# KohakuBlueleaf/UwUDiff

Measured on AMD Instinct MI355X. Metric: train images/sec (whole node), DiT-S/2 256^2 latent, higher is better.
Workload: dtype bf16; 1 GPU; DiT-S/2 (L12 D384 h6), 4x32x32 synthetic latents + pooled-text cond 1280, eps-MSE, AdamW lr1e-6 wd0.01 cosine; random-init weights; per_gpu_batch=768, global_batch=768, parallelism=dp1

## Files before the change

include/uwu_hip.h:

```cpp
#ifndef UWU_HIP_H
#define UWU_HIP_H

#include <stddef.h>
#include <stdint.h>

#ifdef __cplusplus
extern "C" {
#endif

#define UWU_F32 0
#define UWU_BF16 1

#define UWU_OK 0
#define UWU_EINVAL (-1)
#define UWU_ELAUNCH (-2)
#define UWU_ENOTIMPL (-3)

#define UWU_PT_EPSILON 0
#define UWU_PT_V 1
#define UWU_PT_SAMPLE 2
#define UWU_PT_RF 3

#define UWU_EPI_NONE 0
#define UWU_EPI_BIAS 1
#define UWU_EPI_BIAS_GELU 2
#define UWU_EPI_DGELU 3
#define UWU_EPI_BIAS_SILU 4
#define UWU_EPI_ACCUM 5

const char* uwu_last_error(void);
int uwu_version(void);
int uwu_env_refresh(void);
int uwu_memset_zero(void* p, uint64_t bytes, void* stream);


int uwu_schedule_gather(const int64_t* timesteps, const float* sigmas_desc, const float* all_snr,
                        const float* alphas_cumprod, int n_train, int B, int snr_mode, float gamma,
                        int debias, float* coef, void* stream);

int uwu_rf_time_to_sigma(const float* u01, float sigma_max, const float* log_sigmas_asc, int n_train,
                         int B, float* coef, float* timesteps, void* stream);

int uwu_qsample(const float* x, const float* noise, const float* coef, int B, int64_t n, float* noisy,
                void* noisy_bf16, void* stream);

int uwu_qsample_norm(const float* x, const float* noise, const float* coef, int B, int64_t n, float vae_mean,
                     float vae_std, float* x_norm, float* noisy, void* stream);

int uwu_philox_raw(uint32_t* out, int64_t n_counters, uint64_t seed, uint64_t offset, void* stream);
int uwu_philox_normal(float* out, int64_t n, uint64_t seed, uint64_t offset, void* stream);
int uwu_draw_timesteps(int64_t* timesteps, int n_train, int B, uint64_t seed, uint64_t offset, void* stream);
int uwu_draw_u01(float* u01, int B, uint64_t seed, uint64_t offset, void* stream);
int uwu_qsample_draw(const float* x, const float* coef, int B, int64_t n, int use_norm, float vae_mean, float vae_std,
                     float* x_norm, float* noise, float* noisy, uint64_t seed, uint64_t offset, void* stream);
int uwu_posterior_draw(const float* moments, int ldm, int B, int latent, int64_t HW, float* z, float* mean_out, float* logvar_out,
                       uint64_t seed, uint64_t offset, void* stream);

int uwu_ctx_place(const void* src, int dtype, const int64_t* mask, float* out, int B, int S, int F, int S_total,
                  int F_total, int s_off, int f_off, void* stream);

int uwu_loss_fwd_bwd(const float* x, const float* noise, const float* xt, const void* model_output,
                     int out_dtype, const float* coef, int pred_type, int target_type, int force_convert,
                     int B, int64_t n, float* losses, float* loss_mean, void* grad_out, float* pred,
                     float* target, void* stream);

int uwu_scale_inplace(void* y, int dtype, int64_t n, const float* scale, void* stream);
int uwu_scale_into(const void* x, void* y, int dtype, int64_t n, const float* scale, void* stream);
int uwu_cast_i64_to_f32(const int64_t* x, float* y, int64_t n, void* stream);

int uwu_aggregate_concat(const void* emb, const int* starts, void* out, int B, int max_n, int64_t unit_bytes,
                         int elem_size, uint64_t pad_bits, void* stream);
int uwu_aggregate_split(const void* cat, const int* starts, void* out, int B, int max_n, int64_t unit_bytes,
                        void* stream);
int uwu_aggregate_first(const void* emb, const int* starts, void* out, int B, int64_t unit_bytes, void* stream);

int uwu_sampler_step(const float* x, const float* eps_cond, const float* eps_uncond, const float* noise, float* out,
                     float* denoised, int64_t n, float cfg, float sigma, float sigma_down, float sigma_up,
                     float s_noise, void* stream);
int uwu_sampler_combine(const float* base, const float* eps_cond, const float* eps_uncond, const float* noise,
                        float* out, int64_t n, float cfg, float a, float b, float c, void* stream);
int uwu_scale_copy(const float* x, float* y, int64_t n, float scale, void* stream);

int uwu_cfg_input(const float* x, float* y, int B, int64_t n, float c_in, void* stream);
int uwu_sampler_combine_draw(const float* base, const float* eps_cond, const float* eps_uncond, float* out, int64_t n, float cfg,
                             float a, float b, float c, uint64_t seed, uint64_t offset, void* stream);
size_t uwu_latent_finish_ws_bytes(int B, int64_t n);
int uwu_latent_finish(const float* x, float* y, int B, int64_t n, int rescale, float vae_std, float vae_mean, void* ws,
                      size_t ws_bytes, void* stream);
int uwu_image_u8(const void* x, int dtype, void* y, int B, int H, int W, void* stream);


int uwu_grad_sqnorm_clip(const float* g, int64_t n, float pre_scale, float max_norm, float* partial,
                         float* out, void* stream);

int uwu_adamw_step(float* p, float* g, float* m, float* v, void* p_bf16, int64_t n, float lr,
                   float beta1, float beta2, float eps, float weight_decay, int step, float pre_scale,
                   const float* clip, int zero_grad, void* stream);

int uwu_cast_f32_to_bf16(const float* src, void* dst, int64_t n, void* stream);
int uwu_cast_bf16_to_f32(const void* src, float* dst, int64_t n, void* stream);

#define UWU_ADAPTER_NORM 0
#define UWU_ADAPTER_LORA 1
#define UWU_ADAPTER_LOKR 2
#define UWU_ADAPTER_LOKR_LOWRANK 3
int uwu_adapter_merge(const float* base, const float* p, const int64_t* table, const int64_t* blk_start, int nseg,
                      int64_t nblocks, float* eff, void* shadow, void* stream);
int uwu_adapter_grad(const float* dw, int64_t N, int64_t K, int kind, const float* p, float* g, int64_t pa, int64_t pb,
                     int64_t pc, int r, int out_k, int in_n, float scale, float* ws, int64_t ws_elems, void* stream);

int uwu_comm_unique_id(void* id128);
int uwu_comm_init(const void* id128, int rank, int world, void** comm);
int uwu_allreduce_flat(void* comm, float* buf, int64_t n, void* stream);
int uwu_comm_destroy(void* comm);


int uwu_gemm(const void* A, const void* B, void* C, void* C2, const float* bias, const void* aux,
             int M, int N, int K, int lda, int ldb, int ldc, int ldaux, int transA, int transB, int dtype,
             int c_dtype, int epilogue, int split_k, void* stream);

#define UWU_FP8_E4M3 0
#define UWU_FP8_E5M2 1
size_t uwu_gemm_fp8_scratch_bytes(int M, int N, int K);
int uwu_gemm_fp8(const void* A, const void* B, void* C, void* C2, const float* bias, const void* aux, int M, int N,
                 int K, int lda, int ldb, int ldc, int ldaux, int fmt_a, int epilogue, const float* scale_a,
                 const float* scale_b, void* scratch, size_t scratch_bytes, void* stream);

int uwu_gemm_fp8_emit(const void* A, const void* B, void* C, float* colsum, const float* bias, const void* aux, int M, int N,
                      int K, int lda, int ldb, int ldc, int ldaux, int fmt_a, int epilogue, const float* scale_a,
                      const float* scale_b, void* q8, int ldq, void* q8t, int ldqt, const float* q_scale, float* q_amax,
                      void* stream);

int uwu_conv3x3_implicit_ok(int B, int H, int W, int C, int Cout, int stride, int dtype);
int uwu_conv3x3_fwd(const void* x, const void* w, const float* bias, void* y, int B, int H, int W, int C, int Cout,
                    int stride, int dtype, void* stream);
size_t uwu_conv3x3_s2br_ws_bytes(int B, int H, int W, int C, int Cout, int dtype);
int uwu_conv3x3_s2br_fwd(const void* x, const void* w, const float* bias, void* y, int B, int H, int W, int C, int Cout, int dtype,
                         void* ws, size_t ws_bytes, void* stream);
int uwu_conv3x3_dgrad(const void* dy, const void* w, void* dx, int B, int H, int W, int C, int Cout, int stride, int dtype,
                      void* stream);
size_t uwu_conv3x3_wgrad_scratch_bytes(int C, int Cout, int64_t Mo);
int uwu_conv3x3_wgrad(const void* dy, const void* x, float* dw, float* db, int B, int H, int W, int C, int Cout, int stride,
                      int dtype, void* scratch, size_t scratch_bytes, void* stream);

int uwu_fp8_amax(const void* x, int dtype, int64_t n, float* amax, void* stream);
int uwu_fp8_update_scales(float* amax, float* scale, const int* fmt, int n, float margin, void* stream);
int uwu_fp8_quantize(const void* x, int dtype, int M, int K, int ldx, const float* scale, int fmt, void* out, int ldo,
                     void* out_t, int ldt, float* amax, float* colsum, void* stream);

size_t uwu_gemm_wgrad_scratch_bytes(int M, int N, int K);
int uwu_gemm_wgrad(const void* A, const void* B, float* C, float* bias_grad, int M, int N, int K, int lda, int ldb,
                   int ldc, int dtype, int blocks, void* scratch, size_t scratch_bytes, void* stream);

size_t uwu_gemm_wgrad_pair_scratch_bytes(int M_a, int N_a, int M_b, int N_b, int K);
int uwu_gemm_wgrad_pair(const void* A_a, const void* B_a, float* C_a, float* bias_grad_a, int M_a, int N_a, int lda_a,
                        int ldb_a, int ldc_a, const void* A_b, const void* B_b, float* C_b, float* bias_grad_b, int M_b,
                        int N_b, int lda_b, int ldb_b, int ldc_b, int K, int dtype, int blocks, void* scratch,
                        size_t scratch_bytes, void* stream);

int uwu_gemm_prof_enable(int on);
int uwu_gemm_prof_collect(int kind, double* ms, double* flops, int* launches);

enum {
  UWU_PROF_GEMM_FWD = 0, UWU_PROF_GEMM_DGRAD = 1, UWU_PROF_GEMM_WGRAD = 2, UWU_PROF_GEMM_FC1_GELU = 3,
  UWU_PROF_GEMM_FC2_DGELU = 4, UWU_PROF_ATTN_FWD = 5, UWU_PROF_ATTN_BWD = 6, UWU_PROF_LN_FWD = 7, UWU_PROF_LN_BWD = 8,
  UWU_PROF_CONV = 9, UWU_PROF_OTHER = 10
};
int uwu_prof_enable(int on);
int uwu_prof_collect(int tag, int kind, double* ms, double* flops, double* bytes, int* launches);

int uwu_colsum(const void* X, int dtype, int M, int N, int ldx, float* out, int accumulate, void* stream);

int uwu_skinny_linear_ok(int M, int N, int K);
int uwu_skinny_linear_fwd(const float* X, const float* W, const float* bias, float* Y, float* Y2, int M, int N, int K,
                          int epilogue, void* stream);
int uwu_skinny_linear_dgrad(const float* dY, const float* W, float* dX, int M, int N, int K, void* stream);
int uwu_skinny_linear_wgrad(const float* dY, const float* X, float* dW, float* db, int M, int N, int K, void* stream);
int uwu_colsum_batched(const void* X, int dtype, int batch, int M, int N, int ldx, float* out, int accumulate,
                       void* stream);


int uwu_add_ln_modulate_fwd(const void* x_in, const void* y, const float* gate, const float* shift,
                            const float* scale, int mod_ld, void* x_out, void* h, float* mean, float* rstd,
                            int B, int T, int D, float eps, int affine, int dtype, void* stream);
int uwu_add_ln_modulate_fwd_q8(const void* x_in, const void* y, const float* gate, const float* shift, const float* scale,
                               int mod_ld, void* x_out, void* q8, int ldq, void* q8t, int ldqt, const float* q_scale,
                               float* q_amax, float* mean, float* rstd, int B, int T, int D, float eps, void* stream);


int uwu_add_ln_modulate_bwd(const void* dh, const void* x, const float* mean, const float* rstd,
                            const float* scale, const void* dx_in, const void* y, const float* gate,
                            int mod_ld, void* dx_out, void* dy, float* dshift, float* dscale, float* dgate,
                            int B, int T, int D, int affine, int dtype, void* stream);


int uwu_attention_fwd(const void* q, const void* k, const void* v, void* o, float* lse, int B, int Tq, int Tk,
                      int H, int d, int ldq, int ldk, int ldv, int ldo, float scale, int dtype, void* stream);
int uwu_attention_d512_fwd(const void* q, const void* k, const void* v, void* o, int B, int T, int ldq, int ldk, int ldv, int ldo,
                           float scale, int dtype, void* stream);
int uwu_attention_causal_fwd(const void* q, const void* k, const void* v, const int64_t* key_mask, void* o, int B, int T, int H,
                             int d, int ldq, int ldk, int ldv, int ldo, float scale, int dtype, void* stream);
int uwu_text_embed(const int64_t* ids, const void* tok_table, const void* pos_table, void* out, int B, int T, int D, int vocab,
                   int dtype, void* stream);
#define UWU_ACT_QUICK_GELU 0
#define UWU_ACT_GELU_ERF 1
int uwu_bias_act_fwd(const void* x, const float* bias, void* y, int M, int N, int ld, int kind, int dtype, void* stream);
int uwu_text_pool(const int64_t* ids, const void* h, void* pooled, int B, int T, int D, int eos_id, int dtype, void* stream);
int uwu_attention_relbias_fwd(const void* q, const void* k, const void* v, const float* rel_bias, const int64_t* key_mask, void* o,
                              int B, int T, int H, int d, int ldq, int ldk, int ldv, int ldo, float scale, int dtype, void* stream);
int uwu_add_rmsnorm_fwd(const void* x_in, const void* y, const float* weight, void* x_out, void* n_out, int M, int D, float eps,
                        int dtype, void* stream);
#define UWU_GATE_GELU_TANH 0
int uwu_gated_act_fwd(const void* u, void* out, int M, int F, int ldu, int ldo, int kind, int dtype, void* stream);
int uwu_t5_rel_bias(const float* weight, const int32_t* bucket, float* out, int num_buckets, int H, int n, void* stream);
int uwu_token_embed(const int64_t* ids, const void* tok_table, void* out, int B, int T, int D, int vocab, int dtype, void* stream);
int uwu_attention_bwd(const void* q, const void* k, const void* v, const void* o, const void* dO,
                      const float* lse, float* delta, void* dq, void* dk, void* dv, int B, int Tq, int Tk, int H,
                      int d, int ldq, int ldk, int ldv, int ldo, float scale, int dtype, void* stream);
int uwu_attention_bias_fwd(const void* q, const void* k, const void* v, const float* key_bias, void* o, float* lse,
                           int B, int Tq, int Tk, int H, int d, int ldq, int ldk, int ldv, int ldo, float scale,
                           int dtype, void* stream);
int uwu_attention_bias_bwd(const void* q, const void* k, const void* v, const float* key_bias, const void* o,
                           const void* dO, const float* lse, float* delta, void* dq, void* dk, void* dv, int B,
                           int Tq, int Tk, int H, int d, int ldq, int ldk, int ldv, int ldo, float scale, int dtype,
                           void* stream);

int uwu_axial_rope_fwd(const void* x, const float* pos, const float* fh, const float* fw, void* y, int64_t rows,
                       int H, int d, int ldx, int dtype, void* stream);
int uwu_axial_rope_bwd(const void* x, const void* dy, const float* pos, const float* fh, const float* fw, void* dx,
                       float* dfh, float* dfw, int64_t rows, int H, int d, int ldx, int dtype, void* stream);

int uwu_axial_rope_bwd_shared(const void* x, const void* dy, const float* pos, int pos_rows, const float* fh, const float* fw,
                              void* dx, float* dfh, float* dfw, int64_t rows, int H, int d, int ldx, int dtype, void* stream);
int uwu_axial_rope_table(const float* pos, const float* fh, const float* fw, float* tab, int T, int H, int d, int ldt,
                         void* stream);
int uwu_attention_rope_fwd(const void* q, const void* k, const void* v, const float* rope_tab, void* o, float* lse, int B,
                           int T, int H, int d, int ldq, int ldk, int ldv, int ldo, int ldt, float scale, int dtype,
                           void* stream);
int uwu_attention_rope_bwd(const void* q, const void* k, const void* v, const float* rope_tab, const void* o, const void* dO,
                           const float* lse, void* dq, void* dk, void* dv, int B, int T, int H, int d, int ldq, int ldk,
                           int ldv, int ldo, int ldt, float scale, int dtype, void* stream);


int uwu_timestep_embedding(const float* t, int B, int dim, float max_period, void* out, int dtype,
                           void* stream);
int uwu_silu_fwd(const void* x, void* y, int64_t n, int dtype, void* stream);
int uwu_silu_bwd(const void* x, const void* dy, void* dx, int64_t n, int dtype, void* stream);

int uwu_add(const void* a, const void* b, void* out, int64_t n, int dtype, void* stream);
int uwu_transpose_bf16(const void* src, void* dst, int rows, int cols, int ld_src, int ld_dst, void* stream);

int uwu_patchify(const float* img, void* tok, int B, int C, int H, int W, int p, int dtype, void* stream);
int uwu_unpatchify(const void* tok, int dtype, float* img, int B, int C, int H, int W, int p, void* stream);
int uwu_add_pos(void* x, const float* pos, int B, int T, int D, int dtype, void* stream);


int uwu_groupnorm_fwd(const void* x, const float* gamma, const float* beta, void* y, float* mean, float* rstd,
                      int B, int HW, int C, int G, float eps, int silu, int dtype, void* stream);
size_t uwu_groupnorm_fwd_det_ws_bytes(int B, int HW, int C, int G);
int uwu_groupnorm_fwd_det(const void* x, const float* gamma, const float* beta, void* y, float* mean, float* rstd, void* ws,
                          size_t ws_bytes, int B, int HW, int C, int G, float eps, int silu, int dtype, void* stream);
int uwu_groupnorm_bwd(const void* dy, const void* x, const float* mean, const float* rstd, const float* gamma,
                      const float* beta, void* dx, float* dgamma, float* dbeta, float* ws, int B, int HW, int C, int G,
                      int silu, int dtype, void* stream);
int uwu_im2col3x3(const void* x, void* col, int B, int H, int W, int C, int stride, int dtype, void* stream);
int uwu_col2im3x3(const void* dcol, void* dx, int B, int H, int W, int C, int stride, int dtype, void* stream);
int uwu_geglu_fwd(const void* hg, void* out, int64_t M, int F, int dtype, void* stream);
int uwu_geglu_bwd(const void* hg, const void* dout, void* dhg, int64_t M, int F, int dtype, void* stream);
int uwu_upsample2x(const void* src, void* dst, int B, int H, int W, int C, int backward, int dtype, void* stream);
int uwu_add_rowvec(void* x, const void* v, int B, int HW, int C, int dtype, void* stream);
int uwu_nchw_to_cl(const float* nchw, void* cl, int B, int C, int HW, int dtype, void* stream);
int uwu_cl_to_nchw(const void* cl, float* nchw, int B, int C, int HW, int dtype, void* stream);


typedef struct uwu_dit_desc {
  int32_t B, T, D, H, L, mlp_ratio, in_ch, out_ch, patch, img, dtype, cond_dim, freq_dim;
  float ln_eps;
  int32_t mod_total;
  const void* w;
  const float* w32;
  float* g32;
  int64_t off_patch_w, off_patch_b, off_t_w1, off_t_b1, off_t_w2, off_t_b2, off_y_w, off_y_b,
      off_mod_w, off_mod_b, off_final_w, off_final_b;
  int64_t off_layer0, layer_stride;
  const float* pos;
  void* ws;
  size_t ws_bytes;
  void* const* layer_done;
  void* side_stream;
  int32_t rope;
  int64_t off_rope_h, off_rope_w;
  const float* pos_xy;
  int32_t fp8;
  float* f8_scale;
  float* f8_amax;
  const int32_t* f8_fmt;
  int32_t checkpoint;
} uwu_dit_desc;

size_t uwu_dit_workspace_bytes(const uwu_dit_desc* d);
int uwu_dit_forward(const uwu_dit_desc* d, const float* noisy, const float* t, const float* cond,
                    float* out, void* stream);
int uwu_dit_backward(const uwu_dit_desc* d, const float* dout, void* stream);
int uwu_dit_backward_cond(const uwu_dit_desc* d, const float* cond, void* stream);
int64_t uwu_dit_layer_param_stride(int D, int mlp_ratio);

#ifdef __cplusplus
}
#endif
#endif
```

uwudiff_amd/csrc/dit.cpp:

```cpp
#include <hip/hip_runtime.h>
#include <math.h>
#include <stddef.h>
#include <stdint.h>
#include <stdlib.h>

#include "../../include/uwu_hip.h"
#include "env.h"

void uwu_set_error(const char* fmt, ...);

namespace {

constexpr int WGRAD_BLOCKS = 512;

struct Layout {
  size_t es;
  int64_t M, D, D3, D4, Kp, Ko;
  size_t feat, t_pre, t_h, temb, yemb, c, sc, mod;
  size_t sc16, dmod16;
  size_t tok, xe;
  size_t layer0, layer_stride;
  bool ckpt;
  size_t keep, scratch0;
  size_t o_x0, o_m1, o_r1, o_h1, o_qkv, o_lse, o_ao, o_y1, o_x1, o_m2, o_r2, o_h2, o_u, o_f, o_y2;
  size_t o_rope;
  size_t o_h1t, o_aot, o_h2t, o_ft;
  size_t xF, mF, rF, hF, otok;
  size_t dx, dy, dh, dqkv, dao, du, delta, dotok, dmod, dsc, dc, dth, dtp;
  size_t w2t;
  size_t wsc, wsc_bytes;
  size_t x8, x8t, dy8, dy8t, w8, w8_layer;
  size_t total;
};

inline size_t al(size_t x) { return (x + 255) & ~(size_t)255; }

Layout make_layout(const uwu_dit_desc& d) {
  Layout L{};
  L.es = d.dtype == UWU_BF16 ? 2 : 4;
  L.M = (int64_t)d.B * d.T;
  L.D = d.D;
  L.D3 = 3 * (int64_t)d.D;
  L.D4 = (int64_t)d.mlp_ratio * d.D;
  L.Kp = (int64_t)d.in_ch * d.patch * d.patch;
  L.Ko = (int64_t)d.out_ch * d.patch * d.patch;
  size_t p = 0;
  auto take = [&](size_t bytes) { size_t o = p; p = al(p + bytes); return o; };
  const size_t f4 = 4;
  L.feat = take((size_t)d.B * d.freq_dim * f4);
  L.t_pre = take((size_t)d.B * d.D * f4);
  L.t_h = take((size_t)d.B * d.D * f4);
  L.temb = take((size_t)d.B * d.D * f4);
  L.yemb = take((size_t)d.B * d.D * f4);
  L.c = take((size_t)d.B * d.D * f4);
  L.sc = take((size_t)d.B * d.D * f4);
  L.mod = take((size_t)d.B * d.mod_total * f4);
  L.sc16 = take((size_t)d.B * d.D * 2);
  L.dmod16 = take((size_t)d.B * d.mod_total * 2);
  L.tok = take(L.M * L.Kp * L.es);
  L.xe = take(L.M * L.D * L.es);
  size_t q = 0;
  auto sub = [&](size_t bytes) { size_t o = q; q = al(q + bytes); return o; };
  L.o_x0 = sub(L.M * L.D * L.es);
  L.o_m1 = sub(L.M * f4);
  L.o_r1 = sub(L.M * f4);
  L.o_h1 = sub(L.M * L.D * L.es);
  L.o_qkv = sub(L.M * L.D3 * L.es);
  L.o_lse = sub((size_t)d.B * d.H * d.T * f4);
  L.o_ao = sub(L.M * L.D * L.es);
  L.o_y1 = sub(L.M * L.D * L.es);
  L.o_x1 = sub(L.M * L.D * L.es);
  L.o_m2 = sub(L.M * f4);
  L.o_r2 = sub(L.M * f4);
  L.o_h2 = sub(L.M * L.D * L.es);
  L.o_u = sub(L.M * L.D4 * L.es);
  L.o_f = sub(L.M * L.D4 * L.es);
  L.o_y2 = sub(L.M * L.D * L.es);
  if (d.rope) L.o_rope = sub((size_t)d.T * d.D * f4);
  if (d.fp8) {
    L.o_h1t = sub(L.M * L.D);
    L.o_aot = sub(L.M * L.D);
    L.o_h2t = sub(L.M * L.D);
    L.o_ft = sub(L.M * L.D4);
  }
  L.keep = L.o_h1;
  L.ckpt = d.checkpoint != 0;
  L.layer_stride = L.ckpt ? L.keep : q;
  L.layer0 = p;
  p += (size_t)d.L * L.layer_stride;
  if (L.ckpt) L.scratch0 = take(q);
  L.xF = take(L.M * L.D * L.es);
  L.mF = take(L.M * f4);
  L.rF = take(L.M * f4);
  L.hF = take(L.M * L.D * L.es);
  L.otok = take(L.M * L.Ko * L.es);
  L.dx = take(L.M * L.D * L.es);
  L.dy = take(L.M * L.D * L.es);
  L.dh = take(L.M * L.D * L.es);
  L.dqkv = take(L.M * L.D3 * L.es);
  L.dao = take(L.M * L.D * L.es);
  L.du = take(L.M * L.D4 * L.es);
  L.w2t = take((size_t)L.D4 * d.D * 2);
  L.delta = take((size_t)d.B * d.H * d.T * f4);
  L.dotok = take(L.M * L.Ko * L.es);
  L.dmod = take((size_t)d.B * d.mod_total * f4);
  L.dsc = take((size_t)d.B * d.D * f4);
  L.dc = take((size_t)d.B * d.D * f4);
  L.dth = take((size_t)d.B * d.D * f4);
  L.dtp = take((size_t)d.B * d.D * f4);
  L.wsc_bytes = uwu_gemm_wgrad_scratch_bytes((int)L.D4, d.D, (int)L.M);
  for (const size_t t : {uwu_gemm_wgrad_scratch_bytes(d.D, (int)L.D4, (int)L.M),
                         uwu_gemm_wgrad_scratch_bytes((int)L.D3, d.D, (int)L.M),
                         uwu_gemm_wgrad_scratch_bytes(d.D, d.D, (int)L.M),
                         uwu_gemm_wgrad_pair_scratch_bytes((int)L.D4, d.D, d.D, (int)L.D4, (int)L.M),
                         uwu_gemm_wgrad_pair_scratch_bytes((int)L.D3, d.D, d.D, d.D, (int)L.M)})
    if (t > L.wsc_bytes) L.wsc_bytes = t;
  if (d.fp8) {
    for (const size_t t : {uwu_gemm_fp8_scratch_bytes((int)L.D4, d.D, (int)L.M), uwu_gemm_fp8_scratch_bytes(d.D, (int)L.D4, (int)L.M),
                           uwu_gemm_fp8_scratch_bytes((int)L.D3, d.D, (int)L.M), uwu_gemm_fp8_scratch_bytes(d.D, d.D, (int)L.M)})
      if (t > L.wsc_bytes) L.wsc_bytes = t;
  }
  L.wsc_bytes = (L.wsc_bytes + 255) & ~(size_t)255;
  L.wsc = take(L.wsc_bytes * (L.M <= 16384 ? 4 : 1));
  if (d.fp8) {
    L.x8 = take(L.M * L.D4);
    L.x8t = 0;
    L.dy8 = take(L.M * L.D4);
    L.dy8t = take(L.M * L.D4);
    L.w8_layer = al((size_t)24 * d.D * d.D);
    L.w8 = take((size_t)d.L * L.w8_layer);
  }
  L.total = p;
  return L;
}

int check_desc(const uwu_dit_desc* d) {
  if (!d) { uwu_set_error("dit: null descriptor"); return UWU_EINVAL; }
  if (d->B <= 0 || d->T <= 0 || d->D <= 0 || d->H <= 0 || d->L <= 0 || d->D % d->H || d->D % 8 ||
      d->img % d->patch || (d->img / d->patch) * (d->img / d->patch) != d->T || d->mlp_ratio <= 0 ||
      d->freq_dim <= 0 || d->freq_dim % 8) {
    uwu_set_error("dit: inconsistent shape B=%d T=%d D=%d H=%d L=%d img=%d patch=%d", d->B, d->T, d->D, d->H, d->L,
                  d->img, d->patch);
    return UWU_EINVAL;
  }
  if (d->dtype != UWU_F32 && d->dtype != UWU_BF16) { uwu_set_error("dit: bad dtype"); return UWU_EINVAL; }
  if (d->mod_total != d->L * 6 * d->D + 2 * d->D) { uwu_set_error("dit: mod_total mismatch"); return UWU_EINVAL; }
  if ((d->in_ch * d->patch * d->patch) % 8 || (d->out_ch * d->patch * d->patch) % 8 || (d->cond_dim % 8)) {
    uwu_set_error("dit: C*p*p and cond_dim must be multiples of 8");
    return UWU_EINVAL;
  }
  if (!d->w || !d->w32 || !d->pos || !d->ws) { uwu_set_error("dit: null buffer"); return UWU_EINVAL; }
  if (d->rope && (d->dtype != UWU_BF16 || d->D / d->H != 64 || d->T % 64 || d->T > 256 || !d->pos_xy)) {
    uwu_set_error("dit: the fused axial-RoPE attention needs bf16, head dim 64, T a multiple of 64 up to 256 and pos_xy");
    return UWU_EINVAL;
  }
  if (d->fp8) {
    if (d->fp8 < 0 || d->fp8 > 2 || d->dtype != UWU_BF16 || d->D % 128 || d->mlp_ratio != 4 || ((int64_t)d->B * d->T) % 128 ||
        !d->f8_scale || !d->f8_amax || !d->f8_fmt) {
      uwu_set_error("dit: fp8 mode needs bf16 activations, D %% 128 == 0, B*T %% 128 == 0, mlp_ratio 4 and the scale / amax / fmt arrays");
      return UWU_EINVAL;
    }
  }
  return UWU_OK;
}

#define RUN(expr)              \
  do {                         \
    int rc_ = (expr);          \
    if (rc_ != UWU_OK) return rc_; \
  } while (0)

int lin_fwd(const void* X, const void* W, const float* bias, void* Y, void* Y2, int M, int N, int K, int dt, int cdt,
            int epi, void* st) {
  return uwu_gemm(X, W, Y, Y2, bias, nullptr, M, N, K, K, K, N, 0, 0, 0, dt, cdt, epi, 1, st);
}
int lin_fwd32(const float* X, const float* W, const float* bias, float* Y, float* Y2, int M, int N, int K, int epi, void* st) {
  if (M <= 16 && N <= 4096 && uwu_skinny_linear_ok(M, N, K)) return uwu_skinny_linear_fwd(X, W, bias, Y, Y2, M, N, K, epi, st);
  return lin_fwd(X, W, bias, Y, Y2, M, N, K, UWU_F32, UWU_F32, epi, st);
}
int lin_dgrad(const void* dY, const void* W, void* dX, const void* aux, int M, int N, int K, int dt, void* st,
              float* colsum = nullptr) {
  return uwu_gemm(dY, W, dX, colsum, nullptr, aux, M, K, N, N, K, K, K, 0, 1, dt, dt,
                  aux ? UWU_EPI_DGELU : UWU_EPI_NONE, 1, st);
}
static bool mod_bf16(const uwu_dit_desc& d) {
  return d.dtype == UWU_BF16 && d.B >= 64 && d.mod_total % 8 == 0;
}
int lin_dgrad_splitk(const void* dY, const void* W, float* dX, int M, int N, int K, void* st) {
  if (hipMemsetAsync(dX, 0, (size_t)M * K * sizeof(float), (hipStream_t)st) != hipSuccess) {
    uwu_set_error("dgrad_splitk: memset failed");
    return UWU_ELAUNCH;
  }
  const int tiles = ((M + 127) / 128) * ((K + 127) / 128);
  const int ktiles = (N + 31) / 32;
  int split = (512 + tiles - 1) / tiles;
  if (split > ktiles) split = ktiles;
  return uwu_gemm(dY, W, dX, nullptr, nullptr, nullptr, M, K, N, N, K, K, 0, 0, 1, UWU_F32, UWU_F32, UWU_EPI_ACCUM, split,
                  st);
}
int lin_wgrad(const void* dY, const void* X, float* dW, int M, int N, int K, int dt, void* st, void* scratch = nullptr,
              size_t scratch_bytes = 0, float* db = nullptr) {
  if (dt == UWU_BF16 && scratch && uwu_gemm_wgrad_scratch_bytes(N, K, M) <= scratch_bytes)
    return uwu_gemm_wgrad(dY, X, dW, db, N, K, M, N, K, K, dt, WGRAD_BLOCKS, scratch, scratch_bytes, st);
  if (db) {
    const int rc = uwu_colsum(dY, dt, M, N, N, db, 1, st);
    if (rc != UWU_OK) return rc;
  }
  const int tiles = ((N + 127) / 128) * ((K + 127) / 128);
  const int bk = dt == UWU_BF16 ? 64 : 32;
  const int ktiles = (M + bk - 1) / bk;
  const int target = tiles >= 16 ? 768 : 256;
  int split = (target + tiles - 1) / tiles;
  if (split > ktiles) split = ktiles;
  if (split < 1) split = 1;
  return uwu_gemm(dY, X, dW, nullptr, nullptr, nullptr, N, K, M, N, K, K, 0, 1, 1, dt, UWU_F32, UWU_EPI_ACCUM, split, st);
}

bool wgrad_pair_ok(int M, int Na, int Ka, int Nb, int Kb, size_t scratch_bytes) {
  const size_t need = uwu_gemm_wgrad_pair_scratch_bytes(Na, Ka, Nb, Kb, M);
  return need && need <= scratch_bytes;
}
int lin_wgrad_pair(const void* dYa, const void* Xa, float* dWa, float* dba, int Na, int Ka, const void* dYb, const void* Xb,
                   float* dWb, float* dbb, int Nb, int Kb, int M, void* st, void* scratch, size_t scratch_bytes) {
  return uwu_gemm_wgrad_pair(dYa, Xa, dWa, dba, Na, Ka, Na, Ka, Ka, dYb, Xb, dWb, dbb, Nb, Kb, Nb, Kb, Kb, M, UWU_BF16,
                             WGRAD_BLOCKS, scratch, scratch_bytes, st);
}

int lin_wgrad32(const float* dY, const float* X, float* dW, float* db, int M, int N, int K, void* st) {
  if (M <= 16 && uwu_skinny_linear_ok(M, N, K)) return uwu_skinny_linear_wgrad(dY, X, dW, db, M, N, K, st);
  RUN(lin_wgrad(dY, X, dW, M, N, K, UWU_F32, st));
  return uwu_colsum(dY, UWU_F32, M, N, N, db, 1, st);
}

struct F8 {
  int mode;
  float* scale;
  float* amax;
  const int32_t* fmt;
  char *x8, *x8t, *dy8, *dy8t, *wsc, *w8;
  size_t wsc_bytes, w8_layer;
  int D;
  void* st;
  int role(int l, int r) const { return 12 * l + r; }
  char* w(int l, int i, bool t) const {
    static const int off[4] = {0, 6, 8, 16}, sz[4] = {3, 1, 4, 4};
    return w8 + (size_t)l * w8_layer + ((size_t)off[i] + (t ? sz[i] : 0)) * D * D;
  }
  int quant(const void* x, int dtype, int M, int K, int role, void* out, void* out_t, float* colsum, bool have_scale) const {
    const int fm = role % 12 >= 4 && role % 12 < 8 ? UWU_FP8_E5M2 : UWU_FP8_E4M3;
    if (!have_scale && mode == 1) {
      RUN(uwu_fp8_amax(x, dtype, (int64_t)M * K, amax + role, st));
      RUN(uwu_fp8_update_scales(amax + role, scale + role, fmt + role, 1, 1.f, st));
    }
    return uwu_fp8_quantize(x, dtype, M, K, K, scale + role, fm, out, K, out_t, M,
                            (!have_scale && mode == 2) ? amax + role : nullptr, colsum, st);
  }
};

int f8_fwd(const F8& f, const void* X, void* Xt_save, const void* W8, const float* bias, void* Y, void* Y2, int M, int N, int K,
           int rx, int rw, int epi) {
  if (X) RUN(f.quant(X, UWU_BF16, M, K, rx, f.x8, Xt_save, nullptr, false));
  return uwu_gemm_fp8(f.x8, W8, Y, Y2, bias, nullptr, M, N, K, K, K, N, 0, UWU_FP8_E4M3, epi, f.scale + rx, f.scale + rw,
                      nullptr, 0, f.st);
}
int f8_bwd(const F8& f, const void* dY, const void* X8t, const void* W8t, float* dW, float* db, void* dX, const void* aux,
           float* dcol, int M, int N, int K, int rdy, int rx, int rw, const void* dY8 = nullptr, const void* dY8t = nullptr,
           int rnext = -1, void* q8 = nullptr, void* q8t = nullptr) {
  if (dY) {
    RUN(f.quant(dY, UWU_BF16, M, N, rdy, f.dy8, f.dy8t, db, false));
    dY8 = f.dy8;
    dY8t = f.dy8t;
  }
  RUN(uwu_gemm_fp8(dY8t, X8t, dW, nullptr, nullptr, nullptr, N, K, M, M, M, K, 0, UWU_FP8_E5M2, UWU_EPI_ACCUM,
                   f.scale + rdy, f.scale + rx, f.wsc, f.wsc_bytes, f.st));
  if (rnext >= 0)
    return uwu_gemm_fp8_emit(dY8, W8t, nullptr, dcol, nullptr, aux, M, K, N, N, N, K, K, UWU_FP8_E5M2, UWU_EPI_DGELU, f.scale + rdy,
                             f.scale + rw, q8, K, q8t, M, f.scale + rnext, f.amax + rnext, f.st);
  if (!dX) return UWU_OK;
  return uwu_gemm_fp8(dY8, W8t, dX, dcol, nullptr, aux, M, K, N, N, N, K, K, UWU_FP8_E5M2, aux ? UWU_EPI_DGELU : UWU_EPI_NONE,
                      f.scale + rdy, f.scale + rw, nullptr, 0, f.st);
}
static bool f8_emit(const uwu_dit_desc& d);
static int ln_fwd_f8(const uwu_dit_desc& d, const F8& f, const void* x_in, const void* y, const float* gate, const float* shift,
                     const float* scale, int ML, void* x_out, void* h, void* h8t, int role, float* mean, float* rstd, void* st) {
  const int64_t M = (int64_t)d.B * d.T;
  if (f8_emit(d) && d.D <= 1536 && M % 64 == 0) {
    const int rc = uwu_add_ln_modulate_fwd_q8(x_in, y, gate, shift, scale, ML, x_out, f.x8, d.D, h8t, (int)M, f.scale + role,
                                              f.amax + role, mean, rstd, d.B, d.T, d.D, d.ln_eps, st);
    return rc == UWU_OK ? 1 : rc;
  }
  const int rc = uwu_add_ln_modulate_fwd(x_in, y, gate, shift, scale, ML, x_out, h, mean, rstd, d.B, d.T, d.D, d.ln_eps, 0, d.dtype, st);
  return rc == UWU_OK ? 0 : rc;
}
static bool f8_emit(const uwu_dit_desc& d) {
  static UwuEnv on("UWU_F8_EMIT");
  return !on.get().is('0') && d.fp8 == 2;
}

struct Fork {
  hipStream_t main;
  hipStream_t side[4];
  hipEvent_t ev[8];
  bool on = false;
};
bool fork_resources(Fork& f, hipStream_t caller_side) {
  static hipEvent_t pool[8];
  static hipStream_t extra[3];
  static bool made = false;
  if (!made) {
    for (auto& e : pool)
      if (hipEventCreateWithFlags(&e, hipEventDisableTiming | hipEventReleaseToDevice) != hipSuccess) return false;
    for (auto& x : extra)
      if (hipStreamCreateWithFlags(&x, hipStreamNonBlocking) != hipSuccess) return false;
    made = true;
  }
  for (int i = 0; i < 8; ++i) f.ev[i] = pool[i];
  static int n_side = -1;
  if (n_side < 0) {
    const char* e = getenv("UWU_DIT_SIDE_STREAMS");
    n_side = e ? atoi(e) : 1;
    if (n_side < 1 || n_side > 4) n_side = 1;
  }
  for (int i = 0; i < 3; ++i) f.side[i] = n_side == 1 ? caller_side : extra[i % (n_side - 1)];
  f.side[3] = caller_side;
  return true;
}
template <typename F>
int on_side(const Fork& f, int slot, F&& fn) {
  if (!f.on) return fn(static_cast<void*>(f.main), 0);
  if (hipEventRecord(f.ev[slot], f.main) != hipSuccess || hipStreamWaitEvent(f.side[slot], f.ev[slot], 0) != hipSuccess) {
    uwu_set_error("dit_backward: stream fork failed");
    return UWU_ELAUNCH;
  }
  const int rc = fn(static_cast<void*>(f.side[slot]), f.side[slot] == f.side[3] ? 0 : slot + 1);
  if (rc != UWU_OK) return rc;
  if (hipEventRecord(f.ev[4 + slot], f.side[slot]) != hipSuccess) { uwu_set_error("dit_backward: stream fork failed"); return UWU_ELAUNCH; }
  return UWU_OK;
}
int join_side(const Fork& f, int slot) {
  if (f.on && hipStreamWaitEvent(f.main, f.ev[4 + slot], 0) != hipSuccess) {
    uwu_set_error("dit_backward: stream join failed");
    return UWU_ELAUNCH;
  }
  return UWU_OK;
}

struct Ptrs {
  char* ws;
  const Layout& L;
  template <typename T = void>
  T* at(size_t off) const { return reinterpret_cast<T*>(ws + off); }
  template <typename T = void>
  T* lay(int l, size_t sub) const {
    if (L.ckpt && sub >= L.keep) return reinterpret_cast<T*>(ws + L.scratch0 + sub);
    return reinterpret_cast<T*>(ws + L.layer0 + (size_t)l * L.layer_stride + sub);
  }
};

struct LayerW {
  const void *qkv_w, *o_w, *fc1_w, *fc2_w;
  const float *qkv_b, *o_b, *fc1_b, *fc2_b;
  int64_t off_qkv_w, off_qkv_b, off_o_w, off_o_b, off_fc1_w, off_fc1_b, off_fc2_w, off_fc2_b;
};

inline int64_t pad64(int64_t n) { return (n + 63) & ~(int64_t)63; }

LayerW layer_weights(const uwu_dit_desc& d, int l) {
  LayerW w{};
  const int64_t D = d.D, D4 = (int64_t)d.mlp_ratio * d.D;
  int64_t o = d.off_layer0 + (int64_t)l * d.layer_stride;
  w.off_qkv_w = o; o += pad64(3 * D * D);
  w.off_qkv_b = o; o += pad64(3 * D);
  w.off_o_w = o; o += pad64(D * D);
  w.off_o_b = o; o += pad64(D);
  w.off_fc1_w = o; o += pad64(D4 * D);
  w.off_fc1_b = o; o += pad64(D4);
  w.off_fc2_w = o; o += pad64(D * D4);
  w.off_fc2_b = o; o += pad64(D);
  const size_t es = d.dtype == UWU_BF16 ? 2 : 4;
  const char* wb = static_cast<const char*>(d.w);
  w.qkv_w = wb + w.off_qkv_w * es;
  w.o_w = wb + w.off_o_w * es;
  w.fc1_w = wb + w.off_fc1_w * es;
  w.fc2_w = wb + w.off_fc2_w * es;
  w.qkv_b = d.w32 + w.off_qkv_b;
  w.o_b = d.w32 + w.off_o_b;
  w.fc1_b = d.w32 + w.off_fc1_b;
  w.fc2_b = d.w32 + w.off_fc2_b;
  return w;
}


int block_forward(const uwu_dit_desc& d, const Layout& L, const Ptrs& P, const F8& f8, int l, bool recompute, void* st) {
  const int dt = d.dtype, B = d.B, T = d.T, D = d.D, M = (int)L.M, D3 = (int)L.D3, D4 = (int)L.D4;
  const size_t es = L.es;
  const float* w32 = d.w32;
  const int ML = d.mod_total;
  const float* mod = P.at<float>(L.mod);
  const float scale = 1.f / sqrtf((float)(D / d.H));
  const LayerW w = layer_weights(d, l);
  const float* m = mod + (int64_t)l * 6 * D;
  void* x0 = P.lay(l, L.o_x0);
  int h1q = 0, h2q = 0;
  if (d.fp8) {
    if (l == 0 || recompute) {
      h1q = ln_fwd_f8(d, f8, x0, nullptr, nullptr, m + 0, m + D, ML, x0, P.lay(l, L.o_h1), P.lay(l, L.o_h1t), f8.role(l, 0),
                      P.lay<float>(l, L.o_m1), P.lay<float>(l, L.o_r1), st);
    } else {
      const float* mp = mod + (int64_t)(l - 1) * 6 * D;
      h1q = ln_fwd_f8(d, f8, P.lay(l - 1, L.o_x1), P.lay(l - 1, L.o_y2), mp + 5 * D, m + 0, m + D, ML, x0, P.lay(l, L.o_h1),
                      P.lay(l, L.o_h1t), f8.role(l, 0), P.lay<float>(l, L.o_m1), P.lay<float>(l, L.o_r1), st);
    }
    if (h1q < 0) return h1q;
  } else
  if (l == 0 || recompute) {
    RUN(uwu_add_ln_modulate_fwd(x0, nullptr, nullptr, m + 0, m + D, ML, x0, P.lay(l, L.o_h1),
                                P.lay<float>(l, L.o_m1), P.lay<float>(l, L.o_r1), B, T, D, d.ln_eps, 0, dt, st));
  } else {
    const float* mp = mod + (int64_t)(l - 1) * 6 * D;
    RUN(uwu_add_ln_modulate_fwd(P.lay(l - 1, L.o_x1), P.lay(l - 1, L.o_y2), mp + 5 * D, m + 0, m + D, ML, x0,
                                P.lay(l, L.o_h1), P.lay<float>(l, L.o_m1), P.lay<float>(l, L.o_r1), B, T, D,
                                d.ln_eps, 0, dt, st));
  }
  if (d.fp8) RUN(f8_fwd(f8, h1q ? nullptr : P.lay(l, L.o_h1), P.lay(l, L.o_h1t), f8.w(l, 0, false), w.qkv_b, P.lay(l, L.o_qkv), nullptr, M, D3, D, f8.role(l, 0), f8.role(l, 8), UWU_EPI_BIAS));
  else RUN(lin_fwd(P.lay(l, L.o_h1), w.qkv_w, w.qkv_b, P.lay(l, L.o_qkv), nullptr, M, D3, D, dt, dt, UWU_EPI_BIAS, st));
  char* qkv = P.lay<char>(l, L.o_qkv);
  if (d.rope) {
    const int64_t fo = (int64_t)l * d.H * (D / d.H / 4);
    RUN(uwu_axial_rope_table(d.pos_xy, w32 + d.off_rope_h + fo, w32 + d.off_rope_w + fo, P.lay<float>(l, L.o_rope), T, d.H,
                             D / d.H, D, st));
    RUN(uwu_attention_rope_fwd(qkv, qkv + (size_t)D * es, qkv + (size_t)2 * D * es, P.lay<float>(l, L.o_rope), P.lay(l, L.o_ao),
                               P.lay<float>(l, L.o_lse), B, T, d.H, D / d.H, D3, D3, D3, D, D, scale, dt, st));
  } else
  RUN(uwu_attention_fwd(qkv, qkv + (size_t)D * es, qkv + (size_t)2 * D * es, P.lay(l, L.o_ao), P.lay<float>(l, L.o_lse),
                        B, T, T, d.H, D / d.H, D3, D3, D3, D, scale, dt, st));
  if (d.fp8) RUN(f8_fwd(f8, P.lay(l, L.o_ao), P.lay(l, L.o_aot), f8.w(l, 1, false), w.o_b, P.lay(l, L.o_y1), nullptr, M, D, D, f8.role(l, 1), f8.role(l, 9), UWU_EPI_BIAS));
  else RUN(lin_fwd(P.lay(l, L.o_ao), w.o_w, w.o_b, P.lay(l, L.o_y1), nullptr, M, D, D, dt, dt, UWU_EPI_BIAS, st));
  if (d.fp8) {
    h2q = ln_fwd_f8(d, f8, x0, P.lay(l, L.o_y1), m + 2 * D, m + 3 * D, m + 4 * D, ML, P.lay(l, L.o_x1), P.lay(l, L.o_h2),
                    P.lay(l, L.o_h2t), f8.role(l, 2), P.lay<float>(l, L.o_m2), P.lay<float>(l, L.o_r2), st);
    if (h2q < 0) return h2q;
  } else
  RUN(uwu_add_ln_modulate_fwd(x0, P.lay(l, L.o_y1), m + 2 * D, m + 3 * D, m + 4 * D, ML, P.lay(l, L.o_x1),
                              P.lay(l, L.o_h2), P.lay<float>(l, L.o_m2), P.lay<float>(l, L.o_r2), B, T, D, d.ln_eps,
                              0, dt, st));
  if (d.fp8) {
    if (f8_emit(d)) {
      const int r2 = f8.role(l, 2), r3 = f8.role(l, 3);
      if (!h2q) RUN(f8.quant(P.lay(l, L.o_h2), UWU_BF16, M, D, r2, f8.x8, P.lay(l, L.o_h2t), nullptr, false));
      RUN(uwu_gemm_fp8_emit(f8.x8, f8.w(l, 2, false), P.lay(l, L.o_u), nullptr, w.fc1_b, nullptr, M, D4, D, D, D, D4, 0, UWU_FP8_E4M3,
                            UWU_EPI_BIAS_GELU, f8.scale + r2, f8.scale + f8.role(l, 10), f8.dy8, D4, P.lay(l, L.o_ft), M, f8.scale + r3,
                            f8.amax + r3, st));
      RUN(uwu_gemm_fp8(f8.dy8, f8.w(l, 3, false), P.lay(l, L.o_y2), nullptr, w.fc2_b, nullptr, M, D, D4, D4, D4, D, 0, UWU_FP8_E4M3,
                       UWU_EPI_BIAS, f8.scale + r3, f8.scale + f8.role(l, 11), nullptr, 0, st));
      return UWU_OK;
    }
    RUN(f8_fwd(f8, h2q ? nullptr : P.lay(l, L.o_h2), P.lay(l, L.o_h2t), f8.w(l, 2, false), w.fc1_b, P.lay(l, L.o_u), P.lay(l, L.o_f), M, D4, D, f8.role(l, 2), f8.role(l, 10), UWU_EPI_BIAS_GELU));
    RUN(f8_fwd(f8, P.lay(l, L.o_f), P.lay(l, L.o_ft), f8.w(l, 3, false), w.fc2_b, P.lay(l, L.o_y2), nullptr, M, D, D4, f8.role(l, 3), f8.role(l, 11), UWU_EPI_BIAS));
  } else {
    RUN(lin_fwd(P.lay(l, L.o_h2), w.fc1_w, w.fc1_b, P.lay(l, L.o_u), P.lay(l, L.o_f), M, D4, D, dt, dt,
                UWU_EPI_BIAS_GELU, st));
    RUN(lin_fwd(P.lay(l, L.o_f), w.fc2_w, w.fc2_b, P.lay(l, L.o_y2), nullptr, M, D, D4, dt, dt, UWU_EPI_BIAS, st));
  }
  return UWU_OK;
}

}

extern "C" size_t uwu_dit_workspace_bytes(const uwu_dit_desc* d) {
  if (!d) return 0;
  return make_layout(*d).total;
}

extern "C" int64_t uwu_dit_layer_param_stride(int D, int mlp_ratio) {
  const int64_t d = D, d4 = (int64_t)mlp_ratio * D;
  return pad64(3 * d * d) + pad64(3 * d) + pad64(d * d) + pad64(d) + pad64(d4 * d) + pad64(d4) + pad64(d * d4) + pad64(d);
}

extern "C" int uwu_dit_forward(const uwu_dit_desc* dp, const float* noisy, const float* t, const float* cond,
                               float* out, void* st) {
  RUN(check_desc(dp));
  const uwu_dit_desc& d = *dp;
  if (!noisy || !t || !out) { uwu_set_error("dit_forward: null tensor"); return UWU_EINVAL; }
  if ((d.cond_dim > 0) != (cond != nullptr)) { uwu_set_error("dit_forward: cond / cond_dim mismatch"); return UWU_EINVAL; }
  const Layout L = make_layout(d);
  if (d.ws_bytes < L.total) { uwu_set_error("dit_forward: workspace too small (%zu < %zu)", d.ws_bytes, L.total); return UWU_EINVAL; }
  if (d.layer_stride != uwu_dit_layer_param_stride(d.D, d.mlp_ratio)) { uwu_set_error("dit: layer_stride mismatch"); return UWU_EINVAL; }
  Ptrs P{static_cast<char*>(d.ws), L};
  const int dt = d.dtype, B = d.B, T = d.T, D = d.D, M = (int)L.M, D3 = (int)L.D3, D4 = (int)L.D4;
  const size_t es = L.es;
  const char* wb = static_cast<const char*>(d.w);
  const float* w32 = d.w32;
  const int ML = d.mod_total;

  RUN(uwu_timestep_embedding(t, B, d.freq_dim, 10000.f, P.at(L.feat), UWU_F32, st));
  RUN(lin_fwd32(P.at<float>(L.feat), w32 + d.off_t_w1, w32 + d.off_t_b1, P.at<float>(L.t_pre), P.at<float>(L.t_h), B, D,
                d.freq_dim, UWU_EPI_BIAS_SILU, st));
  RUN(lin_fwd32(P.at<float>(L.t_h), w32 + d.off_t_w2, w32 + d.off_t_b2, P.at<float>(L.temb), nullptr, B, D, D, UWU_EPI_BIAS, st));
  const void* cptr = P.at(L.temb);
  if (cond) {
    RUN(lin_fwd32(cond, w32 + d.off_y_w, w32 + d.off_y_b, P.at<float>(L.yemb), nullptr, B, D, d.cond_dim, UWU_EPI_BIAS, st));
    RUN(uwu_add(P.at(L.temb), P.at(L.yemb), P.at(L.c), (int64_t)B * D, UWU_F32, st));
    cptr = P.at(L.c);
  }
  RUN(uwu_silu_fwd(cptr, P.at(L.sc), (int64_t)B * D, UWU_F32, st));
  if (mod_bf16(d)) {
    RUN(uwu_cast_f32_to_bf16(P.at<float>(L.sc), P.at(L.sc16), (int64_t)B * D, st));
    RUN(lin_fwd(P.at(L.sc16), wb + d.off_mod_w * es, w32 + d.off_mod_b, P.at(L.mod), nullptr, B, ML, D, UWU_BF16, UWU_F32, UWU_EPI_BIAS, st));
  } else {
    RUN(lin_fwd32(P.at<float>(L.sc), w32 + d.off_mod_w, w32 + d.off_mod_b, P.at<float>(L.mod), nullptr, B, ML, D, UWU_EPI_BIAS, st));
  }
  const float* mod = P.at<float>(L.mod);

  const F8 f8{d.fp8, d.f8_scale, d.f8_amax, d.f8_fmt, P.at<char>(L.x8), nullptr, P.at<char>(L.dy8),
              P.at<char>(L.dy8t), P.at<char>(L.wsc), P.at<char>(L.w8), L.wsc_bytes, L.w8_layer, d.D, st};
  if (d.fp8) {
    const F8 fw{2, d.f8_scale, d.f8_amax, d.f8_fmt, nullptr, nullptr, nullptr, nullptr, nullptr, f8.w8, 0, L.w8_layer, d.D, st};
    const int rows[4] = {D3, D, D4, D}, cols[4] = {D, D, D, D4};
    for (int l = 0; l < d.L; ++l) {
      const LayerW w = layer_weights(d, l);
      const void* ws4[4] = {w.qkv_w, w.o_w, w.fc1_w, w.fc2_w};
      for (int i = 0; i < 4; ++i)
        RUN(uwu_fp8_amax(ws4[i], UWU_BF16, (int64_t)rows[i] * cols[i], d.f8_amax + fw.role(l, 8 + i), st));
    }
    RUN(uwu_fp8_update_scales(d.f8_amax, d.f8_scale, d.f8_fmt, 12 * d.L, 1.f, st));
    for (int l = 0; l < d.L; ++l) {
      const LayerW w = layer_weights(d, l);
      const void* ws4[4] = {w.qkv_w, w.o_w, w.fc1_w, w.fc2_w};
      for (int i = 0; i < 4; ++i)
        RUN(fw.quant(ws4[i], UWU_BF16, rows[i], cols[i], fw.role(l, 8 + i), fw.w(l, i, false), fw.w(l, i, true), nullptr, true));
    }
  }

  RUN(uwu_patchify(noisy, P.at(L.tok), B, d.in_ch, d.img, d.img, d.patch, dt, st));
  RUN(lin_fwd(P.at(L.tok), wb + d.off_patch_w * es, w32 + d.off_patch_b, P.lay(0, L.o_x0), nullptr, M, D, (int)L.Kp, dt,
              dt, UWU_EPI_BIAS, st));
  RUN(uwu_add_pos(P.lay(0, L.o_x0), d.pos, B, T, D, dt, st));

  for (int l = 0; l < d.L; ++l) RUN(block_forward(d, L, P, f8, l, false, st));
  {
    const int l = d.L - 1;
    const float* mp = mod + (int64_t)l * 6 * D;
    const float* mf = mod + (int64_t)d.L * 6 * D;
    RUN(uwu_add_ln_modulate_fwd(P.lay(l, L.o_x1), P.lay(l, L.o_y2), mp + 5 * D, mf + 0, mf + D, ML, P.at(L.xF),
                                P.at(L.hF), P.at<float>(L.mF), P.at<float>(L.rF), B, T, D, d.ln_eps, 0, dt, st));
    RUN(lin_fwd(P.at(L.hF), wb + d.off_final_w * es, w32 + d.off_final_b, P.at(L.otok), nullptr, M, (int)L.Ko, D, dt, dt,
                UWU_EPI_BIAS, st));
    RUN(uwu_unpatchify(P.at(L.otok), dt, out, B, d.out_ch, d.img, d.img, d.patch, st));
  }
  return UWU_OK;
}

extern "C" int uwu_dit_backward(const uwu_dit_desc* dp, const float* dout, void* st) {
  RUN(check_desc(dp));
  const uwu_dit_desc& d = *dp;
  if (!dout || !d.g32) { uwu_set_error("dit_backward: null tensor"); return UWU_EINVAL; }
  const Layout L = make_layout(d);
  if (d.ws_bytes < L.total) { uwu_set_error("dit_backward: workspace too small"); return UWU_EINVAL; }
  Ptrs P{static_cast<char*>(d.ws), L};
  const int dt = d.dtype, B = d.B, T = d.T, D = d.D, M = (int)L.M, D3 = (int)L.D3, D4 = (int)L.D4;
  const size_t es = L.es;
  const char* wb = static_cast<const char*>(d.w);
  const float* w32 = d.w32;
  float* g = d.g32;
  const int ML = d.mod_total;
  const float* mod = P.at<float>(L.mod);
  float* dmod = P.at<float>(L.dmod);
  if (hipMemsetAsync(dmod, 0, (size_t)B * ML * sizeof(float), (hipStream_t)st) != hipSuccess) {
    uwu_set_error("dit_backward: memset failed");
    return UWU_ELAUNCH;
  }
  const float scale = 1.f / sqrtf((float)(D / d.H));
  const F8 f8{d.fp8, d.f8_scale, d.f8_amax, d.f8_fmt, P.at<char>(L.x8), nullptr, P.at<char>(L.dy8),
              P.at<char>(L.dy8t), P.at<char>(L.wsc), P.at<char>(L.w8), L.wsc_bytes, L.w8_layer, d.D, st};
  Fork fk{static_cast<hipStream_t>(st), {}, {}, false};
  fk.on = d.side_stream && d.side_stream != st && !d.fp8 && dt == UWU_BF16 && M <= 16384 && !L.ckpt &&
          fork_resources(fk, static_cast<hipStream_t>(d.side_stream));
  char* const wsc = P.at<char>(L.wsc);
  bool side_used[4] = {false, false, false, false};
  const bool pairs = !fk.on && !d.fp8 && dt == UWU_BF16 && M > 16384 && !L.ckpt;
  const bool pair_fc = pairs && wgrad_pair_ok(M, D4, D, D, D4, L.wsc_bytes);
  const bool pair_attn = pairs && wgrad_pair_ok(M, D3, D, D, D, L.wsc_bytes);

  RUN(uwu_patchify(dout, P.at(L.dotok), B, d.out_ch, d.img, d.img, d.patch, dt, st));
  RUN(lin_wgrad(P.at(L.dotok), P.at(L.hF), g + d.off_final_w, M, (int)L.Ko, D, dt, st));
  RUN(uwu_colsum(P.at(L.dotok), dt, M, (int)L.Ko, (int)L.Ko, g + d.off_final_b, 1, st));
  RUN(lin_dgrad(P.at(L.dotok), wb + d.off_final_w * es, P.at(L.dh), nullptr, M, (int)L.Ko, D, dt, st));
  {
    const int l = d.L - 1;
    const float* mp = mod + (int64_t)l * 6 * D;
    const float* mf = mod + (int64_t)d.L * 6 * D;
    float* dmp = dmod + (int64_t)l * 6 * D;
    float* dmf = dmod + (int64_t)d.L * 6 * D;
    RUN(uwu_add_ln_modulate_bwd(P.at(L.dh), P.at(L.xF), P.at<float>(L.mF), P.at<float>(L.rF), mf + D, nullptr,
                                P.lay(l, L.o_y2), mp + 5 * D, ML, P.at(L.dx), P.at(L.dy), dmf + 0, dmf + D, dmp + 5 * D,
                                B, T, D, 0, dt, st));
  }
  for (int l = d.L - 1; l >= 0; --l) {
    const LayerW w = layer_weights(d, l);
    const float* m = mod + (int64_t)l * 6 * D;
    float* dm = dmod + (int64_t)l * 6 * D;
    if (d.fp8) {
      if (f8_emit(d)) {
        RUN(f8_bwd(f8, P.at(L.dy), P.lay(l, L.o_ft), f8.w(l, 3, true), g + w.off_fc2_w, g + w.off_fc2_b, nullptr, P.lay(l, L.o_u),
                   g + w.off_fc1_b, M, D, D4, f8.role(l, 7), f8.role(l, 3), f8.role(l, 11), nullptr, nullptr, f8.role(l, 6), f8.x8, f8.dy8t));
        RUN(f8_bwd(f8, nullptr, P.lay(l, L.o_h2t), f8.w(l, 2, true), g + w.off_fc1_w, nullptr, P.at(L.dh), nullptr, nullptr, M, D4, D,
                   f8.role(l, 6), f8.role(l, 2), f8.role(l, 10), f8.x8, f8.dy8t));
      } else {
      RUN(f8_bwd(f8, P.at(L.dy), P.lay(l, L.o_ft), f8.w(l, 3, true), g + w.off_fc2_w, g + w.off_fc2_b, P.at(L.du), P.lay(l, L.o_u),
                 g + w.off_fc1_b, M, D, D4, f8.role(l, 7), f8.role(l, 3), f8.role(l, 11)));
      RUN(f8_bwd(f8, P.at(L.du), P.lay(l, L.o_h2t), f8.w(l, 2, true), g + w.off_fc1_w, nullptr, P.at(L.dh), nullptr, nullptr, M, D4, D,
                 f8.role(l, 6), f8.role(l, 2), f8.role(l, 10)));
      }
    } else {
    if (!pair_fc) {
    RUN(on_side(fk, 0, [&](void* s2, int k) {
      return lin_wgrad(P.at(L.dy), P.lay(l, L.o_f), g + w.off_fc2_w, M, D, D4, dt, s2, wsc + (size_t)k * L.wsc_bytes, L.wsc_bytes, g + w.off_fc2_b);
    }));
    side_used[0] = true;
    }
    if (side_used[1]) RUN(join_side(fk, 1));
    if (dt == UWU_BF16 && D == 384 && M % 256 == 0 && M >= 256 * 256 && D4 % 64 == 0 && D4 >= 1024 && D4 <= 2048) {
      RUN(uwu_transpose_bf16(w.fc2_w, P.at(L.w2t), D, D4, D4, D, st));
      RUN(uwu_gemm(P.at(L.dy), P.at(L.w2t), P.at(L.du), nullptr, nullptr, P.lay(l, L.o_u), M, D4, D, D, D, D4, D4, 0, 0, dt, dt,
                   UWU_EPI_DGELU, 1, st));
    } else {
      RUN(lin_dgrad(P.at(L.dy), w.fc2_w, P.at(L.du), P.lay(l, L.o_u), M, D, D4, dt, st, nullptr));
    }
    if (pair_fc) {
      RUN(lin_wgrad_pair(P.at(L.du), P.lay(l, L.o_h2), g + w.off_fc1_w, g + w.off_fc1_b, D4, D, P.at(L.dy), P.lay(l, L.o_f),
                         g + w.off_fc2_w, g + w.off_fc2_b, D, D4, M, st, wsc, L.wsc_bytes));
    } else {
    RUN(on_side(fk, 1, [&](void* s2, int k) {
      return lin_wgrad(P.at(L.du), P.lay(l, L.o_h2), g + w.off_fc1_w, M, D4, D, dt, s2, wsc + (size_t)k * L.wsc_bytes, L.wsc_bytes, g + w.off_fc1_b);
    }));
    side_used[1] = true;
    }
    RUN(lin_dgrad(P.at(L.du), w.fc1_w, P.at(L.dh), nullptr, M, D4, D, dt, st));
    RUN(join_side(fk, 0));
    }
    RUN(uwu_add_ln_modulate_bwd(P.at(L.dh), P.lay(l, L.o_x1), P.lay<float>(l, L.o_m2), P.lay<float>(l, L.o_r2), m + 4 * D,
                                P.at(L.dx), P.lay(l, L.o_y1), m + 2 * D, ML, P.at(L.dx), P.at(L.dy), dm + 3 * D,
                                dm + 4 * D, dm + 2 * D, B, T, D, 0, dt, st));
    if (d.fp8) {
      RUN(f8_bwd(f8, P.at(L.dy), P.lay(l, L.o_aot), f8.w(l, 1, true), g + w.off_o_w, g + w.off_o_b, P.at(L.dao), nullptr, nullptr, M, D, D,
                 f8.role(l, 5), f8.role(l, 1), f8.role(l, 9)));
    } else {
    if (!pair_attn) {
    RUN(on_side(fk, 2, [&](void* s2, int k) {
      return lin_wgrad(P.at(L.dy), P.lay(l, L.o_ao), g + w.off_o_w, M, D, D, dt, s2, wsc + (size_t)k * L.wsc_bytes, L.wsc_bytes, g + w.off_o_b);
    }));
    side_used[2] = true;
    }
    RUN(lin_dgrad(P.at(L.dy), w.o_w, P.at(L.dao), nullptr, M, D, D, dt, st));
    if (side_used[3]) RUN(join_side(fk, 3));
    }
    char* qkv = P.lay<char>(l, L.o_qkv);
    char* dqkv = P.at<char>(L.dqkv);
    if (d.rope) {
      const int64_t fo = (int64_t)l * d.H * (D / d.H / 4);
      RUN(uwu_attention_rope_bwd(qkv, qkv + (size_t)D * es, qkv + (size_t)2 * D * es, P.lay<float>(l, L.o_rope), P.lay(l, L.o_ao),
                                 P.at(L.dao), P.lay<float>(l, L.o_lse), dqkv, dqkv + (size_t)D * es, dqkv + (size_t)2 * D * es,
                                 B, T, d.H, D / d.H, D3, D3, D3, D, D, scale, dt, st));
      for (int qk = 0; qk < 2; ++qk)
        RUN(uwu_axial_rope_bwd_shared(qkv + (size_t)qk * D * es, dqkv + (size_t)qk * D * es, d.pos_xy, T,
                                      w32 + d.off_rope_h + fo, w32 + d.off_rope_w + fo, dqkv + (size_t)qk * D * es,
                                      g + d.off_rope_h + fo, g + d.off_rope_w + fo, (int64_t)M, d.H, D / d.H, D3, dt, st));
    } else
    RUN(uwu_attention_bwd(qkv, qkv + (size_t)D * es, qkv + (size_t)2 * D * es, P.lay(l, L.o_ao), P.at(L.dao),
                          P.lay<float>(l, L.o_lse), P.at<float>(L.delta), dqkv, dqkv + (size_t)D * es,
                          dqkv + (size_t)2 * D * es, B, T, T, d.H, D / d.H, D3, D3, D3, D, scale, dt, st));
    if (d.fp8) {
      RUN(f8_bwd(f8, dqkv, P.lay(l, L.o_h1t), f8.w(l, 0, true), g + w.off_qkv_w, g + w.off_qkv_b, P.at(L.dh), nullptr, nullptr, M, D3, D,
                 f8.role(l, 4), f8.role(l, 0), f8.role(l, 8)));
    } else if (pair_attn) {
      RUN(lin_wgrad_pair(dqkv, P.lay(l, L.o_h1), g + w.off_qkv_w, g + w.off_qkv_b, D3, D, P.at(L.dy), P.lay(l, L.o_ao),
                         g + w.off_o_w, g + w.off_o_b, D, D, M, st, wsc, L.wsc_bytes));
    } else {
    RUN(on_side(fk, 3, [&](void* s2, int k) {
      return lin_wgrad(dqkv, P.lay(l, L.o_h1), g + w.off_qkv_w, M, D3, D, dt, s2, wsc + (size_t)k * L.wsc_bytes, L.wsc_bytes, g + w.off_qkv_b);
    }));
    side_used[3] = true;
    }
    if (fk.on && d.layer_done && d.layer_done[l])
      for (int k = 0; k < 3; ++k)
        if (fk.side[k] != fk.side[3] && hipStreamWaitEvent(fk.side[3], fk.ev[4 + k], 0) != hipSuccess) {
          uwu_set_error("dit_backward: stream join failed");
          return UWU_ELAUNCH;
        }
    if (d.layer_done && d.layer_done[l] &&
        hipEventRecord(static_cast<hipEvent_t>(d.layer_done[l]), fk.on ? fk.side[3] : static_cast<hipStream_t>(st)) != hipSuccess) {
      uwu_set_error("dit_backward: hipEventRecord(layer_done[%d]) failed", l);
      return UWU_ELAUNCH;
    }
    if (!d.fp8) RUN(lin_dgrad(dqkv, w.qkv_w, P.at(L.dh), nullptr, M, D3, D, dt, st));
    if (!d.fp8) RUN(join_side(fk, 2));
    if (L.ckpt && l > 0) RUN(block_forward(d, L, P, f8, l - 1, true, st));
    if (l > 0) {
      const float* mp = mod + (int64_t)(l - 1) * 6 * D;
      float* dmp = dmod + (int64_t)(l - 1) * 6 * D;
      RUN(uwu_add_ln_modulate_bwd(P.at(L.dh), P.lay(l, L.o_x0), P.lay<float>(l, L.o_m1), P.lay<float>(l, L.o_r1), m + D,
                                  P.at(L.dx), P.lay(l - 1, L.o_y2), mp + 5 * D, ML, P.at(L.dx), P.at(L.dy), dm + 0,
                                  dm + D, dmp + 5 * D, B, T, D, 0, dt, st));
    } else {
      RUN(uwu_add_ln_modulate_bwd(P.at(L.dh), P.lay(l, L.o_x0), P.lay<float>(l, L.o_m1), P.lay<float>(l, L.o_r1), m + D,
                                  P.at(L.dx), nullptr, nullptr, ML, P.at(L.dx), nullptr, dm + 0, dm + D, nullptr, B, T, D, 0, dt, st));
    }
  }
  if (fk.on)
    for (int k = 0; k < 4; ++k) RUN(join_side(fk, k));
  RUN(lin_wgrad(P.at(L.dx), P.at(L.tok), g + d.off_patch_w, M, D, (int)L.Kp, dt, st));
  RUN(uwu_colsum(P.at(L.dx), dt, M, D, D, g + d.off_patch_b, 1, st));

  if (mod_bf16(d)) {
    RUN(uwu_cast_f32_to_bf16(dmod, P.at(L.dmod16), (int64_t)B * ML, st));
    RUN(lin_wgrad(P.at(L.dmod16), P.at(L.sc16), g + d.off_mod_w, B, ML, D, UWU_BF16, st));
    RUN(uwu_colsum(dmod, UWU_F32, B, ML, ML, g + d.off_mod_b, 1, st));
    if (hipMemsetAsync(P.at(L.dsc), 0, (size_t)B * D * sizeof(float), (hipStream_t)st) != hipSuccess) {
      uwu_set_error("dit_backward: memset failed");
      return UWU_ELAUNCH;
    }
    {
      const int tiles = ((B + 127) / 128) * ((D + 127) / 128), ktiles = (ML + 63) / 64;
      int split = (512 + tiles - 1) / tiles;
      if (split > ktiles) split = ktiles;
      RUN(uwu_gemm(P.at(L.dmod16), wb + d.off_mod_w * es, P.at(L.dsc), nullptr, nullptr, nullptr, B, D, ML, ML, D, D, 0, 0, 1, UWU_BF16,
                   UWU_F32, UWU_EPI_ACCUM, split, st));
    }
  } else {
    RUN(lin_wgrad32(dmod, P.at<float>(L.sc), g + d.off_mod_w, g + d.off_mod_b, B, ML, D, st));
    RUN(lin_dgrad_splitk(dmod, w32 + d.off_mod_w, P.at<float>(L.dsc), B, ML, D, st));
  }
  const void* cptr = d.cond_dim > 0 ? P.at(L.c) : P.at(L.temb);
  RUN(uwu_silu_bwd(cptr, P.at(L.dsc), P.at(L.dc), (int64_t)B * D, UWU_F32, st));
  if (d.cond_dim > 0) {
  }
  RUN(lin_wgrad32(P.at<float>(L.dc), P.at<float>(L.t_h), g + d.off_t_w2, g + d.off_t_b2, B, D, D, st));
  if (B <= 16 && uwu_skinny_linear_ok(B, D, D) && D <= 512) RUN(uwu_skinny_linear_dgrad(P.at<float>(L.dc), w32 + d.off_t_w2, P.at<float>(L.dth), B, D, D, st));
  else RUN(lin_dgrad(P.at(L.dc), w32 + d.off_t_w2, P.at(L.dth), nullptr, B, D, D, UWU_F32, st));
  RUN(uwu_silu_bwd(P.at(L.t_pre), P.at(L.dth), P.at(L.dtp), (int64_t)B * D, UWU_F32, st));
  RUN(lin_wgrad32(P.at<float>(L.dtp), P.at<float>(L.feat), g + d.off_t_w1, g + d.off_t_b1, B, D, d.freq_dim, st));
  return UWU_OK;
}

extern "C" int uwu_dit_backward_cond(const uwu_dit_desc* dp, const float* cond, void* st) {
  RUN(check_desc(dp));
  const uwu_dit_desc& d = *dp;
  if (d.cond_dim <= 0) return UWU_OK;
  if (!cond || !d.g32) { uwu_set_error("dit_backward_cond: null tensor"); return UWU_EINVAL; }
  const Layout L = make_layout(d);
  Ptrs P{static_cast<char*>(d.ws), L};
  return lin_wgrad32(P.at<float>(L.dc), cond, d.g32 + d.off_y_w, d.g32 + d.off_y_b, d.B, d.D, d.cond_dim, st);
}
```

uwudiff_amd/csrc/embed.hip:

```cpp
#include "common.h"

namespace {

template <typename T>
__global__ void timestep_embedding_kernel(const float* __restrict__ t, int B, int dim, float max_period,
                                          T* __restrict__ out) {
  const int half = dim >> 1;
  const int i = blockIdx.x * blockDim.x + threadIdx.x;
  if (i >= B * half) return;
  const int b = i / half, j = i - b * half;
  const float f = expf(-logf(max_period) * (float)j / (float)half);
  const float a = t[b] * f;
  out[(int64_t)b * dim + j] = from_f32<T>(cosf(a));
  out[(int64_t)b * dim + half + j] = from_f32<T>(sinf(a));
}

template <typename T>
__global__ void silu_fwd_kernel(const T* __restrict__ x, T* __restrict__ y, int64_t n4) {
  const int64_t stride = (int64_t)gridDim.x * blockDim.x;
  for (int64_t i = (int64_t)blockIdx.x * blockDim.x + threadIdx.x; i < n4; i += stride) {
    f32x4 v = load4(x + 4 * i);
#pragma unroll
    for (int e = 0; e < 4; ++e) v[e] = silu_f(v[e]);
    store4(y + 4 * i, v);
  }
}
template <typename T>
__global__ void silu_bwd_kernel(const T* __restrict__ x, const T* __restrict__ dy, T* __restrict__ dx, int64_t n4) {
  const int64_t stride = (int64_t)gridDim.x * blockDim.x;
  for (int64_t i = (int64_t)blockIdx.x * blockDim.x + threadIdx.x; i < n4; i += stride) {
    f32x4 v = load4(x + 4 * i), g = load4(dy + 4 * i);
#pragma unroll
    for (int e = 0; e < 4; ++e) g[e] *= dsilu_f(v[e]);
    store4(dx + 4 * i, g);
  }
}

template <typename T, bool TO_TOKENS>
__global__ void patch_kernel(float* __restrict__ img, T* __restrict__ tok, int B, int C, int H, int W, int p) {
  const int gh = H / p, gw = W / p, kp = C * p * p;
  const int64_t total = (int64_t)B * gh * gw * kp;
  const int64_t stride = (int64_t)gridDim.x * blockDim.x;
  for (int64_t i = (int64_t)blockIdx.x * blockDim.x + threadIdx.x; i < total; i += stride) {
    int64_t m = i / kp;
    int k = (int)(i - m * kp);
    int tw = (int)(m % gw);
    int64_t r = m / gw;
    int th = (int)(r % gh);
    int b = (int)(r / gh);
    int pw = k % p, ph = (k / p) % p, c = k / (p * p);
    int64_t src = (((int64_t)b * C + c) * H + (th * p + ph)) * W + (tw * p + pw);
    if (TO_TOKENS)
      tok[i] = from_f32<T>(img[src]);
    else
      img[src] = to_f32(tok[i]);
  }
}

template <typename T>
__global__ void add_kernel(const T* __restrict__ a, const T* __restrict__ b, T* __restrict__ o, int64_t n4) {
  const int64_t stride = (int64_t)gridDim.x * blockDim.x;
  for (int64_t i = (int64_t)blockIdx.x * blockDim.x + threadIdx.x; i < n4; i += stride)
    store4(o + 4 * i, load4(a + 4 * i) + load4(b + 4 * i));
}

template <typename T>
__global__ void add_pos_kernel(T* __restrict__ x, const float* __restrict__ pos, int64_t total4, int64_t td4) {
  const int64_t stride = (int64_t)gridDim.x * blockDim.x;
  for (int64_t i = (int64_t)blockIdx.x * blockDim.x + threadIdx.x; i < total4; i += stride) {
    f32x4 v = load4(x + 4 * i), pv = load4(pos + 4 * (i % td4));
    store4(x + 4 * i, v + pv);
  }
}

}

#define DISPATCH_T(dtype, NAME, ...)                                                    \
  if ((dtype) == UWU_F32) { NAME(float, __VA_ARGS__); }                                  \
  else if ((dtype) == UWU_BF16) { NAME(bf16_t, __VA_ARGS__); }                           \
  else { uwu_set_error("bad dtype %d", (int)(dtype)); return UWU_EINVAL; }

extern "C" int uwu_timestep_embedding(const float* t, int B, int dim, float max_period, void* out, int dtype,
                                      void* stream) {
  UWU_CHECK_ARG(t && out && B > 0 && dim > 0 && dim % 2 == 0, "timestep_embedding: bad args");
  hipStream_t st = (hipStream_t)stream;
  const int n = B * dim / 2;
#define TE(T, ...) hipLaunchKernelGGL((timestep_embedding_kernel<T>), dim3(cdiv(n, 256)), dim3(256), 0, st, t, B, dim, max_period, (T*)out)
  DISPATCH_T(dtype, TE, 0)
#undef TE
  UWU_LAUNCH_CHECK("timestep_embedding");
  return UWU_OK;
}

extern "C" int uwu_silu_fwd(const void* x, void* y, int64_t n, int dtype, void* stream) {
  UWU_CHECK_ARG(x && y && n > 0 && n % 4 == 0, "silu_fwd: n must be a positive multiple of 4");
  hipStream_t st = (hipStream_t)stream;
#define SF(T, ...) hipLaunchKernelGGL((silu_fwd_kernel<T>), dim3(ew_grid(n / 4, 256)), dim3(256), 0, st, (const T*)x, (T*)y, n / 4)
  DISPATCH_T(dtype, SF, 0)
#undef SF
  UWU_LAUNCH_CHECK("silu_fwd");
  return UWU_OK;
}

extern "C" int uwu_silu_bwd(const void* x, const void* dy, void* dx, int64_t n, int dtype, void* stream) {
  UWU_CHECK_ARG(x && dy && dx && n > 0 && n % 4 == 0, "silu_bwd: n must be a positive multiple of 4");
  hipStream_t st = (hipStream_t)stream;
#define SB(T, ...) hipLaunchKernelGGL((silu_bwd_kernel<T>), dim3(ew_grid(n / 4, 256)), dim3(256), 0, st, (const T*)x, (const T*)dy, (T*)dx, n / 4)
  DISPATCH_T(dtype, SB, 0)
#undef SB
  UWU_LAUNCH_CHECK("silu_bwd");
  return UWU_OK;
}

extern "C" int uwu_patchify(const float* img, void* tok, int B, int C, int H, int W, int p, int dtype, void* stream) {
  UWU_CHECK_ARG(img && tok && B > 0 && C > 0 && p > 0 && H % p == 0 && W % p == 0, "patchify: bad shape");
  hipStream_t st = (hipStream_t)stream;
  const int64_t total = (int64_t)B * C * H * W;
#define PF(T, ...) hipLaunchKernelGGL((patch_kernel<T, true>), dim3(ew_grid(total, 256)), dim3(256), 0, st, const_cast<float*>(img), (T*)tok, B, C, H, W, p)
  DISPATCH_T(dtype, PF, 0)
#undef PF
  UWU_LAUNCH_CHECK("patchify");
  return UWU_OK;
}

extern "C" int uwu_unpatchify(const void* tok, int dtype, float* img, int B, int C, int H, int W, int p, void* stream) {
  UWU_CHECK_ARG(img && tok && B > 0 && C > 0 && p > 0 && H % p == 0 && W % p == 0, "unpatchify: bad shape");
  hipStream_t st = (hipStream_t)stream;
  const int64_t total = (int64_t)B * C * H * W;
#define UF(T, ...) hipLaunchKernelGGL((patch_kernel<T, false>), dim3(ew_grid(total, 256)), dim3(256), 0, st, img, (T*)const_cast<void*>(tok), B, C, H, W, p)
  DISPATCH_T(dtype, UF, 0)
#undef UF
  UWU_LAUNCH_CHECK("unpatchify");
  return UWU_OK;
}

extern "C" int uwu_add_pos(void* x, const float* pos, int B, int T, int D, int dtype, void* stream) {
  UWU_CHECK_ARG(x && pos && B > 0 && T > 0 && D > 0 && D % 4 == 0, "add_pos: bad args");
  hipStream_t st = (hipStream_t)stream;
  const int64_t td4 = (int64_t)T * D / 4, total4 = td4 * B;
#define AP(T_, ...) hipLaunchKernelGGL((add_pos_kernel<T_>), dim3(ew_grid(total4, 256)), dim3(256), 0, st, (T_*)x, pos, total4, td4)
  DISPATCH_T(dtype, AP, 0)
#undef AP
  UWU_LAUNCH_CHECK("add_pos");
  return UWU_OK;
}

extern "C" int uwu_add(const void* a, const void* b, void* out, int64_t n, int dtype, void* stream) {
  UWU_CHECK_ARG(a && b && out && n > 0 && n % 4 == 0, "add: n must be a positive multiple of 4");
  hipStream_t st = (hipStream_t)stream;
#define AD(T, ...) hipLaunchKernelGGL((add_kernel<T>), dim3(ew_grid(n / 4, 256)), dim3(256), 0, st, (const T*)a, (const T*)b, (T*)out, n / 4)
  DISPATCH_T(dtype, AD, 0)
#undef AD
  UWU_LAUNCH_CHECK("add");
  return UWU_OK;
}

namespace {
__global__ void __launch_bounds__(256) transpose_bf16_kernel(const bf16_t* __restrict__ src, bf16_t* __restrict__ dst, int rows,
                                                             int cols, int lds, int ldd) {
  __shared__ bf16_t tile[32][34];
  const int tx = threadIdx.x & 31, ty = threadIdx.x >> 5;
  const int r0 = blockIdx.y * 32, c0 = blockIdx.x * 32;
#pragma unroll
  for (int k = 0; k < 4; ++k) {
    const int r = r0 + ty + 8 * k, c = c0 + tx;
    tile[ty + 8 * k][tx] = (r < rows && c < cols) ? src[(int64_t)r * lds + c] : (bf16_t)0.f;
  }
  __syncthreads();
#pragma unroll
  for (int k = 0; k < 4; ++k) {
    const int c = c0 + ty + 8 * k, r = r0 + tx;
    if (c < cols && r < rows) dst[(int64_t)c * ldd + r] = tile[tx][ty + 8 * k];
  }
}
}

extern "C" int uwu_transpose_bf16(const void* src, void* dst, int rows, int cols, int ld_src, int ld_dst, void* stream) {
  UWU_CHECK_ARG(src && dst && rows > 0 && cols > 0 && ld_src >= cols && ld_dst >= rows, "transpose_bf16: bad argument");
  hipLaunchKernelGGL(transpose_bf16_kernel, dim3((cols + 31) / 32, (rows + 31) / 32), dim3(256), 0, (hipStream_t)stream,
                     (const bf16_t*)src, (bf16_t*)dst, rows, cols, ld_src, ld_dst);
  UWU_LAUNCH_CHECK("transpose_bf16");
  return UWU_OK;
}
```

uwudiff_amd/csrc/norm.hip:

```cpp
#include "common.h"

namespace {
__device__ __forceinline__ f32x8 load8_nt(const float* p) { return load8(p); }
__device__ __forceinline__ f32x8 load8_nt(const bf16_t* p) {
  typedef unsigned nu32x4 __attribute__((ext_vector_type(4)));
  nu32x4 raw = __builtin_nontemporal_load(reinterpret_cast<const nu32x4*>(p));
  bf16x8 v = *reinterpret_cast<bf16x8*>(&raw);
  f32x8 r;
#pragma unroll
  for (int i = 0; i < 8; ++i) r[i] = (float)v[i];
  return r;
}
__device__ __forceinline__ void store8_nt(float* p, f32x8 v) { store8(p, v); }
__device__ __forceinline__ void store8_nt(bf16_t* p, f32x8 v) {
  typedef unsigned nu32x4 __attribute__((ext_vector_type(4)));
  bf16x8 o;
#pragma unroll
  for (int i = 0; i < 8; ++i) o[i] = (bf16_t)v[i];
  __builtin_nontemporal_store(*reinterpret_cast<nu32x4*>(&o), reinterpret_cast<nu32x4*>(p));
}

template <typename T> struct Raw8;
template <> struct Raw8<float> { typedef f32x8 type; };
template <> struct Raw8<bf16_t> { typedef bf16x8 type; };
__device__ __forceinline__ f32x8 raw8_nt(const float* p) { return load8(p); }
__device__ __forceinline__ bf16x8 raw8_nt(const bf16_t* p) {
  typedef unsigned nu32x4 __attribute__((ext_vector_type(4)));
  nu32x4 raw = __builtin_nontemporal_load(reinterpret_cast<const nu32x4*>(p));
  return *reinterpret_cast<bf16x8*>(&raw);
}
__device__ __forceinline__ f32x8 raw8(const float* p) { return load8(p); }
__device__ __forceinline__ bf16x8 raw8(const bf16_t* p) { return *reinterpret_cast<const bf16x8*>(p); }
__device__ __forceinline__ f32x8 unpack8(f32x8 v) { return v; }
__device__ __forceinline__ f32x8 unpack8(bf16x8 v) {
  f32x8 r;
#pragma unroll
  for (int i = 0; i < 8; ++i) r[i] = (float)v[i];
  return r;
}

constexpr int MAX_D = 4096;

template <typename T, int MAX_IT>
__global__ void __launch_bounds__(256) add_ln_mod_fwd_kernel(const T* __restrict__ x_in, const T* __restrict__ y,
                                                             const float* __restrict__ gate,
                                                             const float* __restrict__ shift,
                                                             const float* __restrict__ scale, int mod_ld,
                                                             T* __restrict__ x_out, T* __restrict__ h,
                                                             float* __restrict__ mean_o, float* __restrict__ rstd_o,
                                                             int M, int T_tok, int D, float eps, int affine) {
  const int lane = threadIdx.x & 63, wave = threadIdx.x >> 6;
  const int nit = (D + 511) >> 9;
  for (int row = blockIdx.x * 4 + wave; row < M; row += gridDim.x * 4) {
    const int b = row / T_tok;
    const int64_t off = (int64_t)row * D;
    f32x8 v[MAX_IT];
    float s = 0.f;
#pragma unroll
    for (int it = 0; it < MAX_IT; ++it) {
      const int d = it * 512 + lane * 8;
      if (it < nit && d < D) {
        f32x8 xv = load8_nt(x_in + off + d);
        if (y) {
          f32x8 yv = load8_nt(y + off + d), gv = load8(gate + (int64_t)b * mod_ld + d);
          xv = xv + gv * yv;
          if constexpr (sizeof(T) == 2) {
#pragma unroll
            for (int e = 0; e < 8; ++e) xv[e] = (float)(bf16_t)xv[e];
          }
          store8_nt(x_out + off + d, xv);
        }
        v[it] = xv;
        _Pragma("unroll") for (int e = 0; e < 8; ++e) s += xv[e];
      } else {
        v[it] = f32x8{0.f, 0.f, 0.f, 0.f, 0.f, 0.f, 0.f, 0.f};
      }
    }
    const float mean = wave_sum(s) / (float)D;
    float q = 0.f;
#pragma unroll
    for (int it = 0; it < MAX_IT; ++it) {
      const int d = it * 512 + lane * 8;
      if (it < nit && d < D) {
#pragma unroll
        for (int e = 0; e < 8; ++e) {
          float c = v[it][e] - mean;
          q += c * c;
        }
      }
    }
    const float var = wave_sum(q) / (float)D;
    const float rstd = 1.f / sqrtf(var + eps);
    if (lane == 0) {
      mean_o[row] = mean;
      rstd_o[row] = rstd;
    }
#pragma unroll
    for (int it = 0; it < MAX_IT; ++it) {
      const int d = it * 512 + lane * 8;
      if (it < nit && d < D) {
        f32x8 o;
#pragma unroll
        for (int e = 0; e < 8; ++e) o[e] = (v[it][e] - mean) * rstd;
        if (scale) {
          f32x8 sc = load8(scale + (int64_t)b * mod_ld + d), sh = load8(shift + (int64_t)b * mod_ld + d);
#pragma unroll
          for (int e = 0; e < 8; ++e) o[e] = o[e] * (affine ? sc[e] : 1.f + sc[e]) + sh[e];
        }
        store8(h + off + d, o);
      }
    }
  }
}

template <typename T, int NCH>
__global__ void __launch_bounds__(256) add_ln_mod_fwd16_kernel(const T* __restrict__ x_in, const T* __restrict__ y,
                                                               const float* __restrict__ gate,
                                                               const float* __restrict__ shift,
                                                               const float* __restrict__ scale, int mod_ld,
                                                               T* __restrict__ x_out, T* __restrict__ h,
                                                               float* __restrict__ mean_o, float* __restrict__ rstd_o,
                                                               int M, int T_tok, float eps, int affine) {
  constexpr int D = 128 * NCH;
  const int lane = threadIdx.x & 63, wave = threadIdx.x >> 6;
  const int sub = lane >> 4, l16 = lane & 15;
  for (int row0 = (blockIdx.x * 4 + wave) * 4; row0 < M; row0 += gridDim.x * 16) {
    const int row = row0 + sub;
    const bool ok = row < M;
    const int rc = ok ? row : M - 1;
    const int b = rc / T_tok;
    const int64_t off = (int64_t)rc * D + 8 * l16;
    const float* gb = gate + (int64_t)b * mod_ld + 8 * l16;
    f32x8 v[NCH];
    float s = 0.f;
#pragma unroll
    for (int cidx = 0; cidx < NCH; ++cidx) {
      f32x8 xv = load8_nt(x_in + off + 128 * cidx);
      if (y) {
        const f32x8 yv = load8_nt(y + off + 128 * cidx), gv = load8(gb + 128 * cidx);
        xv = xv + gv * yv;
        if constexpr (sizeof(T) == 2) {
#pragma unroll
          for (int e = 0; e < 8; ++e) xv[e] = (float)(bf16_t)xv[e];
        }
        if (ok) store8_nt(x_out + off + 128 * cidx, xv);
      }
      v[cidx] = xv;
#pragma unroll
      for (int e = 0; e < 8; ++e) s += xv[e];
    }
    const float mean = row16_sum(s) * (1.f / (float)D);
    float q = 0.f;
#pragma unroll
    for (int cidx = 0; cidx < NCH; ++cidx)
#pragma unroll
      for (int e = 0; e < 8; ++e) {
        const float c = v[cidx][e] - mean;
        q += c * c;
      }
    const float var = row16_sum(q) * (1.f / (float)D);
    const float rstd = 1.f / sqrtf(var + eps);
    if (l16 == 0 && ok) {
      mean_o[row] = mean;
      rstd_o[row] = rstd;
    }
#pragma unroll
    for (int cidx = 0; cidx < NCH; ++cidx) {
      f32x8 o;
#pragma unroll
      for (int e = 0; e < 8; ++e) o[e] = (v[cidx][e] - mean) * rstd;
      if (scale) {
        const f32x8 sc = load8(scale + (int64_t)b * mod_ld + 8 * l16 + 128 * cidx), sh = load8(shift + (int64_t)b * mod_ld + 8 * l16 + 128 * cidx);
#pragma unroll
        for (int e = 0; e < 8; ++e) o[e] = o[e] * (affine ? sc[e] : 1.f + sc[e]) + sh[e];
      }
      if (ok) store8(h + off + 128 * cidx, o);
    }
  }
}

__device__ __forceinline__ unsigned q8_pack4(float a, float b, float c, float d, float s) {
  a = fminf(fmaxf(a * s, -448.f), 448.f);
  b = fminf(fmaxf(b * s, -448.f), 448.f);
  c = fminf(fmaxf(c * s, -448.f), 448.f);
  d = fminf(fmaxf(d * s, -448.f), 448.f);
  int r = __builtin_amdgcn_cvt_pk_fp8_f32(a, b, 0, false);
  return (unsigned)__builtin_amdgcn_cvt_pk_fp8_f32(c, d, r, true);
}

template <int MAX_IT, int NW>
__global__ void __launch_bounds__(64 * NW, 4) add_ln_mod_fwd_q8_kernel(
    const bf16_t* __restrict__ x_in, const bf16_t* __restrict__ y, const float* __restrict__ gate,
    const float* __restrict__ shift, const float* __restrict__ scale, int mod_ld, bf16_t* __restrict__ x_out,
    unsigned char* __restrict__ q8, int ldq, unsigned char* __restrict__ q8t, int ldqt, const float* __restrict__ q_scale,
    float* __restrict__ q_amax, float* __restrict__ mean_o, float* __restrict__ rstd_o, int M, int T_tok, int D, float eps) {
  extern __shared__ __attribute__((aligned(16))) unsigned char img[];
  __shared__ float red[NW];
  const int lane = threadIdx.x & 63, wave = threadIdx.x >> 6;
  const int nit = (D + 511) >> 9;
  const int row0 = blockIdx.x * 8 * NW;
  const int pitch = D + 8;
  const float qs = q_scale[0];
  float mx = 0.f;
  bf16x8 xr[2][MAX_IT], yr[MAX_IT];
  auto fetch = [&](int r, int buf) {
    const int64_t off = (int64_t)(row0 + 8 * wave + r) * D;
#pragma unroll
    for (int it = 0; it < MAX_IT; ++it) {
      const int d = it * 512 + lane * 8;
      if (it < nit && d < D) {
        xr[buf][it] = raw8_nt(x_in + off + d);
        if (y) yr[it] = raw8_nt(y + off + d);
      }
    }
  };
  fetch(0, 0);
#pragma unroll
  for (int r = 0; r < 8; ++r) {
    const int buf = r & 1;
    const int row = row0 + 8 * wave + r;
    const int b = row / T_tok;
    const int64_t off = (int64_t)row * D;
    bf16x8 v[MAX_IT];
    float s = 0.f;
#pragma unroll
    for (int it = 0; it < MAX_IT; ++it) {
      const int d = it * 512 + lane * 8;
      if (it < nit && d < D) {
        f32x8 xv = unpack8(xr[buf][it]);
        v[it] = xr[buf][it];
        if (y) {
          const f32x8 yv = unpack8(yr[it]), gv = load8(gate + (int64_t)b * mod_ld + d);
          xv = xv + gv * yv;
#pragma unroll
          for (int e = 0; e < 8; ++e) v[it][e] = (bf16_t)xv[e];
          typedef unsigned nu32x4 __attribute__((ext_vector_type(4)));
          __builtin_nontemporal_store(*reinterpret_cast<nu32x4*>(&v[it]), reinterpret_cast<nu32x4*>(x_out + off + d));
          xv = unpack8(v[it]);
        }
        _Pragma("unroll") for (int e = 0; e < 8; ++e) s += xv[e];
      }
    }
    if (r + 1 < 8) fetch(r + 1, buf ^ 1);
    const float mean = wave_sum(s) / (float)D;
    float q = 0.f;
#pragma unroll
    for (int it = 0; it < MAX_IT; ++it) {
      const int d = it * 512 + lane * 8;
      if (it < nit && d < D) {
        const f32x8 xv = unpack8(v[it]);
#pragma unroll
        for (int e = 0; e < 8; ++e) {
          float c = xv[e] - mean;
          q += c * c;
        }
      }
    }
    const float var = wave_sum(q) / (float)D;
    const float rstd = 1.f / sqrtf(var + eps);
    if (lane == 0) {
      mean_o[row] = mean;
      rstd_o[row] = rstd;
    }
#pragma unroll
    for (int it = 0; it < MAX_IT; ++it) {
      const int d = it * 512 + lane * 8;
      if (it < nit && d < D) {
        f32x8 o;
        const f32x8 sc = load8(scale + (int64_t)b * mod_ld + d), sh = load8(shift + (int64_t)b * mod_ld + d);
        const f32x8 xv = unpack8(v[it]);
#pragma unroll
        for (int e = 0; e < 8; ++e) {
          o[e] = (xv[e] - mean) * rstd * (1.f + sc[e]) + sh[e];
          mx = fmaxf(mx, fabsf(o[e]));
        }
        const unsigned lo = q8_pack4(o[0], o[1], o[2], o[3], qs), hi = q8_pack4(o[4], o[5], o[6], o[7], qs);
        *reinterpret_cast<uint2*>(q8 + (int64_t)row * ldq + d) = uint2{lo, hi};
        *reinterpret_cast<uint2*>(img + (8 * wave + r) * pitch + d) = uint2{lo, hi};
      }
    }
  }
  mx = wave_max(mx);
  if (lane == 0) red[wave] = mx;
  __syncthreads();
  if (q_amax && threadIdx.x == 0) {
    float a = red[0];
#pragma unroll
    for (int w = 1; w < NW; ++w) a = fmaxf(a, red[w]);
    const unsigned cur = __hip_atomic_load(reinterpret_cast<unsigned*>(q_amax), __ATOMIC_RELAXED, __HIP_MEMORY_SCOPE_AGENT);
    if (__float_as_uint(a) > cur) atomicMax(reinterpret_cast<unsigned*>(q_amax), __float_as_uint(a));
  }
  constexpr int RB = NW / 2;
  const int nq = D >> 2;
  for (int idx = threadIdx.x; idx < RB * nq; idx += 64 * NW) {
    const int cq = idx / RB, rb = idx - cq * RB;
    const unsigned* src = reinterpret_cast<const unsigned*>(img + (16 * rb) * pitch) + cq;
    unsigned w[16];
#pragma unroll
    for (int i = 0; i < 16; ++i) w[i] = src[i * (pitch >> 2)];
#pragma unroll
    for (int e = 0; e < 4; ++e) {
      const unsigned sel = 0x0c0c0400u + (unsigned)e * 0x0101u;
      uint4 o;
      o.x = __builtin_amdgcn_perm(w[1], w[0], sel) | (__builtin_amdgcn_perm(w[3], w[2], sel) << 16);
      o.y = __builtin_amdgcn_perm(w[5], w[4], sel) | (__builtin_amdgcn_perm(w[7], w[6], sel) << 16);
      o.z = __builtin_amdgcn_perm(w[9], w[8], sel) | (__builtin_amdgcn_perm(w[11], w[10], sel) << 16);
      o.w = __builtin_amdgcn_perm(w[13], w[12], sel) | (__builtin_amdgcn_perm(w[15], w[14], sel) << 16);
      *reinterpret_cast<uint4*>(q8t + (int64_t)(4 * cq + e) * ldqt + row0 + 16 * rb) = o;
    }
  }
}

template <typename T, int MAX_IT, int NW = 4>
__global__ void __launch_bounds__(64 * NW) add_ln_mod_bwd_kernel(
    const T* __restrict__ dh, const T* __restrict__ x, const float* __restrict__ mean_i,
    const float* __restrict__ rstd_i, const float* __restrict__ scale, const T* __restrict__ dx_in,
    const T* __restrict__ y, const float* __restrict__ gate, int mod_ld, T* __restrict__ dx_out, T* __restrict__ dy,
    float* __restrict__ dshift, float* __restrict__ dscale, float* __restrict__ dgate, int M, int T_tok, int D,
    int rows_per_block, int affine) {
  extern __shared__ __attribute__((aligned(16))) float red[];
  const int lane = threadIdx.x & 63, wave = threadIdx.x >> 6;
  const int nit = (D + 511) >> 9;
  const int row0 = blockIdx.x * rows_per_block;
  const int b = row0 / T_tok;
  f32x8 a_sh[MAX_IT], a_sc[MAX_IT], a_g[MAX_IT];
#pragma unroll
  for (int it = 0; it < MAX_IT; ++it) a_sh[it] = a_sc[it] = a_g[it] = f32x8{0.f, 0.f, 0.f, 0.f, 0.f, 0.f, 0.f, 0.f};

  for (int r = wave; r < rows_per_block; r += NW) {
    const int row = row0 + r;
    if (row >= M) break;
    const int64_t off = (int64_t)row * D;
    const float mean = mean_i[row], rstd = rstd_i[row];
    if constexpr (MAX_IT == 1) {
      f32x8 xh[MAX_IT], g[MAX_IT];
      float s1 = 0.f, s2 = 0.f;
  #pragma unroll
      for (int it = 0; it < MAX_IT; ++it) {
        const int d = it * 512 + lane * 8;
        if (it < nit && d < D) {
          f32x8 xv = load8_nt(x + off + d), dv = load8(dh + off + d);
          f32x8 sc = scale ? load8(scale + (int64_t)b * mod_ld + d)
                           : (affine ? f32x8{1.f, 1.f, 1.f, 1.f, 1.f, 1.f, 1.f, 1.f} : f32x8{0.f, 0.f, 0.f, 0.f, 0.f, 0.f, 0.f, 0.f});
  #pragma unroll
          for (int e = 0; e < 8; ++e) {
            float xhat = (xv[e] - mean) * rstd;
            float gg = dv[e] * (affine ? sc[e] : 1.f + sc[e]);
            xh[it][e] = xhat;
            g[it][e] = gg;
            s1 += gg;
            s2 += gg * xhat;
            a_sh[it][e] += dv[e];
            a_sc[it][e] += dv[e] * xhat;
          }
        }
      }
      s1 = wave_sum(s1) / (float)D;
      s2 = wave_sum(s2) / (float)D;
  #pragma unroll
      for (int it = 0; it < MAX_IT; ++it) {
        const int d = it * 512 + lane * 8;
        if (it < nit && d < D) {
          f32x8 dx;
  #pragma unroll
          for (int e = 0; e < 8; ++e) dx[e] = rstd * (g[it][e] - s1 - xh[it][e] * s2);
          if (dx_in) dx = dx + load8_nt(dx_in + off + d);
          store8_nt(dx_out + off + d, dx);
          if (y) {
            f32x8 yv = load8_nt(y + off + d), gv = load8(gate + (int64_t)b * mod_ld + d);
            store8(dy + off + d, gv * dx);
  #pragma unroll
            for (int e = 0; e < 8; ++e) a_g[it][e] += dx[e] * yv[e];
          }
        }
      }
    } else {
      typename Raw8<T>::type xr[MAX_IT], dr[MAX_IT];
      float s1 = 0.f, s2 = 0.f;
      auto scale_of = [&](int d) {
        return scale ? load8(scale + (int64_t)b * mod_ld + d)
                     : (affine ? f32x8{1.f, 1.f, 1.f, 1.f, 1.f, 1.f, 1.f, 1.f} : f32x8{0.f, 0.f, 0.f, 0.f, 0.f, 0.f, 0.f, 0.f});
      };
  #pragma unroll
      for (int it = 0; it < MAX_IT; ++it) {
        const int d = it * 512 + lane * 8;
        if (it < nit && d < D) {
          xr[it] = raw8_nt(x + off + d);
          dr[it] = raw8(dh + off + d);
          const f32x8 xv = unpack8(xr[it]), dv = unpack8(dr[it]), sc = scale_of(d);
  #pragma unroll
          for (int e = 0; e < 8; ++e) {
            float xhat = (xv[e] - mean) * rstd;
            float gg = dv[e] * (affine ? sc[e] : 1.f + sc[e]);
            s1 += gg;
            s2 += gg * xhat;
            a_sh[it][e] += dv[e];
            a_sc[it][e] += dv[e] * xhat;
          }
        }
      }
      s1 = wave_sum(s1) / (float)D;
      s2 = wave_sum(s2) / (float)D;
  #pragma unroll
      for (int it = 0; it < MAX_IT; ++it) {
        const int d = it * 512 + lane * 8;
        if (it < nit && d < D) {
          const f32x8 xv = unpack8(xr[it]), dv = unpack8(dr[it]), sc = scale_of(d);
          f32x8 dx;
  #pragma unroll
          for (int e = 0; e < 8; ++e) {
            const float xhat = (xv[e] - mean) * rstd, gg = dv[e] * (affine ? sc[e] : 1.f + sc[e]);
            dx[e] = rstd * (gg - s1 - xhat * s2);
          }
          if (dx_in) dx = dx + load8_nt(dx_in + off + d);
          store8_nt(dx_out + off + d, dx);
          if (y) {
            f32x8 yv = load8_nt(y + off + d), gv = load8(gate + (int64_t)b * mod_ld + d);
            store8(dy + off + d, gv * dx);
  #pragma unroll
            for (int e = 0; e < 8; ++e) a_g[it][e] += dx[e] * yv[e];
          }
        }
      }
    }
  }
  constexpr bool ONE_SLAB = MAX_IT >= 3;
  float* mine = red + (ONE_SLAB ? 0 : (int64_t)wave * 3 * D);
  if constexpr (ONE_SLAB) {
    for (int w = 0; w < NW; ++w) {
      if (wave == w) {
#pragma unroll
        for (int it = 0; it < MAX_IT; ++it) {
          const int d = it * 512 + lane * 8;
          if (it < nit && d < D) {
            if (w == 0) {
              store8(mine + d, a_sh[it]);
              store8(mine + D + d, a_sc[it]);
              store8(mine + 2 * D + d, a_g[it]);
            } else {
              store8(mine + d, load8(mine + d) + a_sh[it]);
              store8(mine + D + d, load8(mine + D + d) + a_sc[it]);
              store8(mine + 2 * D + d, load8(mine + 2 * D + d) + a_g[it]);
            }
          }
        }
      }
      __syncthreads();
    }
  } else {
#pragma unroll
    for (int it = 0; it < MAX_IT; ++it) {
      const int d = it * 512 + lane * 8;
      if (it < nit && d < D) {
        store8(mine + d, a_sh[it]);
        store8(mine + D + d, a_sc[it]);
        store8(mine + 2 * D + d, a_g[it]);
      }
    }
    __syncthreads();
  }
  const int ncol = (y ? 3 : 2) * D;
  for (int c = threadIdx.x; c < ncol; c += 64 * NW) {
    float t = 0.f;
    if constexpr (ONE_SLAB) {
      t = red[c];
    } else {
#pragma unroll
      for (int w = 0; w < NW; ++w) t += red[w * 3 * D + c];
    }
    const int which = c / D, d = c - which * D;
    float* dst = which == 0 ? dshift : (which == 1 ? dscale : dgate);
    if (dst) atomicAdd(dst + (int64_t)b * mod_ld + d, t);
  }
}

template <typename T, int MAX_IT>
__global__ void __launch_bounds__(512) ln_affine_bwd_kernel(
    const T* __restrict__ dh, const T* __restrict__ x, const float* __restrict__ mean_i,
    const float* __restrict__ rstd_i, const float* __restrict__ weight, const T* __restrict__ dx_in,
    T* __restrict__ dx_out, float* __restrict__ dbias, float* __restrict__ dweight, int M, int D, int rows_per_block) {
  extern __shared__ __attribute__((aligned(16))) float red[];
  const int lane = threadIdx.x & 63, wave = threadIdx.x >> 6;
  const int nit = (D + 511) >> 9;
  const int row0 = blockIdx.x * rows_per_block;
  f32x8 a_sh[MAX_IT], a_sc[MAX_IT], wv[MAX_IT];
#pragma unroll
  for (int it = 0; it < MAX_IT; ++it) {
    a_sh[it] = a_sc[it] = f32x8{0.f, 0.f, 0.f, 0.f, 0.f, 0.f, 0.f, 0.f};
    const int d = it * 512 + lane * 8;
    wv[it] = (it < nit && d < D) ? load8(weight + d) : a_sh[it];
  }
  for (int r = wave; r < rows_per_block; r += 8) {
    const int row = row0 + r;
    if (row >= M) break;
    const int64_t off = (int64_t)row * D;
    const float mean = mean_i[row], rstd = rstd_i[row];
    f32x8 xh[MAX_IT], g[MAX_IT], din[MAX_IT];
    float s1 = 0.f, s2 = 0.f;
#pragma unroll
    for (int it = 0; it < MAX_IT; ++it) {
      const int d = it * 512 + lane * 8;
      if (it < nit && d < D) {
        const f32x8 xv = load8_nt(x + off + d), dv = load8(dh + off + d);
        if (dx_in) din[it] = load8_nt(dx_in + off + d);
#pragma unroll
        for (int e = 0; e < 8; ++e) {
          const float xhat = (xv[e] - mean) * rstd, gg = dv[e] * wv[it][e];
          xh[it][e] = xhat;
          g[it][e] = gg;
          s1 += gg;
          s2 += gg * xhat;
          a_sh[it][e] += dv[e];
          a_sc[it][e] += dv[e] * xhat;
        }
      }
    }
    s1 = wave_sum(s1) / (float)D;
    s2 = wave_sum(s2) / (float)D;
#pragma unroll
    for (int it = 0; it < MAX_IT; ++it) {
      const int d = it * 512 + lane * 8;
      if (it < nit && d < D) {
        f32x8 dx;
#pragma unroll
        for (int e = 0; e < 8; ++e) dx[e] = rstd * (g[it][e] - s1 - xh[it][e] * s2);
        if (dx_in) dx = dx + din[it];
        store8_nt(dx_out + off + d, dx);
      }
    }
  }
  float* mine = red + (int64_t)wave * 2 * D;
#pragma unroll
  for (int it = 0; it < MAX_IT; ++it) {
    const int d = it * 512 + lane * 8;
    if (it < nit && d < D) {
      store8(mine + d, a_sh[it]);
      store8(mine + D + d, a_sc[it]);
    }
  }
  __syncthreads();
  for (int c = threadIdx.x; c < 2 * D; c += 512) {
    float t = 0.f;
#pragma unroll
    for (int w = 0; w < 8; ++w) t += red[w * 2 * D + c];
    atomicAdd(c < D ? dbias + c : dweight + (c - D), t);
  }
}

template <typename T>
__global__ void __launch_bounds__(256) colsum_kernel(const T* __restrict__ X, int M, int N, int ldx,
                                                     float* __restrict__ out, int rows_per_block) {
  __shared__ f32x4 red[16][17];
  const int cg = threadIdx.x & 15, rg = threadIdx.x >> 4;
  const int n = blockIdx.x * 64 + cg * 4;
  X += (int64_t)blockIdx.z * M * ldx;
  out += (int64_t)blockIdx.z * N;
  const int r0 = blockIdx.y * rows_per_block;
  int r1 = r0 + rows_per_block;
  if (r1 > M) r1 = M;
  f32x4 a = {0.f, 0.f, 0.f, 0.f};
  if (n < N)
    for (int r = r0 + rg; r < r1; r += 16) a = a + load4(X + (int64_t)r * ldx + n);
  red[rg][cg] = a;
  __syncthreads();
  if (rg == 0 && n < N) {
    f32x4 t = red[0][cg];
#pragma unroll
    for (int i = 1; i < 16; ++i) t = t + red[i][cg];
#pragma unroll
    for (int e = 0; e < 4; ++e) atomicAdd(out + n + e, t[e]);
  }
}

}

extern "C" int uwu_add_ln_modulate_fwd_q8(const void* x_in, const void* y, const float* gate, const float* shift,
                                          const float* scale, int mod_ld, void* x_out, void* q8, int ldq, void* q8t, int ldqt,
                                          const float* q_scale, float* q_amax, float* mean, float* rstd, int B, int T, int D,
                                          float eps, void* stream) {
  UWU_CHECK_ARG(x_in && q8 && q8t && q_scale && mean && rstd && shift && scale, "add_ln_modulate_fwd_q8: null pointer");
  UWU_CHECK_ARG(B > 0 && T > 0 && D > 0 && D % 8 == 0 && D <= 1536, "add_ln_modulate_fwd_q8: D=%d unsupported", D);
  UWU_CHECK_ARG(((int64_t)B * T) % 64 == 0, "add_ln_modulate_fwd_q8: B*T must be a multiple of 64");
  UWU_CHECK_ARG((y == nullptr) || (gate && x_out), "add_ln_modulate_fwd_q8: y needs gate and x_out");
  UWU_CHECK_ARG(mod_ld % 4 == 0, "add_ln_modulate_fwd_q8: mod_ld must be a multiple of 4");
  UWU_CHECK_ARG((((uintptr_t)x_in | (uintptr_t)y | (uintptr_t)x_out | (uintptr_t)q8t) & 15) == 0 && ((uintptr_t)q8 & 7) == 0,
                "add_ln_modulate_fwd_q8: misaligned tensor");
  const int M = B * T;
  UWU_CHECK_ARG(ldq >= D && ldq % 8 == 0 && ldqt >= M && ldqt % 16 == 0, "add_ln_modulate_fwd_q8: bad leading dimension");
  hipStream_t st = (hipStream_t)stream;
  const int nw = (size_t)64 * (D + 8) * 2 <= 150 * 1024 ? 8 : 4;
  UWU_CHECK_ARG(M % (8 * nw) == 0, "add_ln_modulate_fwd_q8: B*T must be a multiple of %d", 8 * nw);
  const size_t lds = (size_t)8 * nw * (D + 8);
  UwuProfScope prof(stream);
#define Q8_LAUNCH(NIT, NW)                                                                                                 \
  {                                                                                                                        \
    static unsigned char done[UWU_MAX_DEV];                                                                                \
    if (!uwu_func_lds(reinterpret_cast<const void*>(add_ln_mod_fwd_q8_kernel<NIT, NW>), 8 * NW * (1536 + 8), done)) {    \
      uwu_set_error("add_ln_modulate_fwd_q8: the device cannot give a workgroup %d bytes of LDS", 8 * NW * (1536 + 8));   \
      return UWU_ELAUNCH;                                                                                                  \
    }                                                                                                                      \
    hipLaunchKernelGGL((add_ln_mod_fwd_q8_kernel<NIT, NW>), dim3(M / (8 * NW)), dim3(64 * NW), lds, st,                   \
                       (const bf16_t*)x_in, (const bf16_t*)y, gate, shift, scale, mod_ld, (bf16_t*)x_out,                 \
                       (unsigned char*)q8, ldq, (unsigned char*)q8t, ldqt, q_scale, q_amax, mean, rstd, M, T, D, eps);     \
  }
#define Q8_CASE(NIT)                \
  case NIT:                         \
    if (nw == 8) Q8_LAUNCH(NIT, 8)  \
    else Q8_LAUNCH(NIT, 4)          \
    break;
  switch ((D + 511) / 512) { Q8_CASE(1) Q8_CASE(2) Q8_CASE(3) }
#undef Q8_CASE
#undef Q8_LAUNCH
  const double md = (double)M * D;
  prof.done(UWU_PROF_LN_FWD, 0, 8.0 * md, md * (2.0 * (1 + (y ? 2 : 0)) + 2.0));
  UWU_LAUNCH_CHECK("add_ln_modulate_fwd_q8");
  return UWU_OK;
}

extern "C" int uwu_add_ln_modulate_fwd(const void* x_in, const void* y, const float* gate, const float* shift,
                                       const float* scale, int mod_ld, void* x_out, void* h, float* mean, float* rstd,
                                       int B, int T, int D, float eps, int affine, int dtype, void* stream) {
  UWU_CHECK_ARG(x_in && h && mean && rstd, "add_ln_modulate_fwd: null pointer");
  UWU_CHECK_ARG(B > 0 && T > 0 && D > 0 && D % 8 == 0 && D <= MAX_D, "add_ln_modulate_fwd: D=%d unsupported", D);
  UWU_CHECK_ARG((y == nullptr) || (gate && x_out), "add_ln_modulate_fwd: y needs gate and x_out");
  UWU_CHECK_ARG((scale == nullptr) == (shift == nullptr), "add_ln_modulate_fwd: scale/shift go together");
  UWU_CHECK_ARG(!scale || mod_ld % 4 == 0, "add_ln_modulate_fwd: mod_ld must be a multiple of 4");
  UWU_CHECK_ARG((((uintptr_t)x_in | (uintptr_t)h) & 15) == 0, "add_ln_modulate_fwd: tensors must be 16-byte aligned");
  const int M = B * T;
  int grid = (M + 3) / 4;
  if (grid > 8192) grid = 8192;
  hipStream_t st = (hipStream_t)stream;
  UWU_CHECK_ARG(dtype == UWU_F32 || dtype == UWU_BF16, "add_ln_modulate_fwd: bad dtype");
  UwuProfScope prof(stream);
  static UwuEnv r16("UWU_LN_ROW16");
  const bool al16 = (((uintptr_t)x_in | (uintptr_t)h | (uintptr_t)y | (uintptr_t)x_out) & 15) == 0 && (mod_ld % 4 == 0);
  if (!r16.get().is('0') && D % 128 == 0 && D <= (r16.get().is('1') ? 1536 : 768) && al16 && M >= 4096) {
    int g16 = (M + 15) / 16;
    if (g16 > 4096) g16 = 4096;
#define F16_CASE(NCH)                                                                                                          \
  case NCH:                                                                                                                    \
    if (dtype == UWU_F32)                                                                                                      \
      hipLaunchKernelGGL((add_ln_mod_fwd16_kernel<float, NCH>), dim3(g16), dim3(256), 0, st, (const float*)x_in, (const float*)y, \
                         gate, shift, scale, mod_ld, (float*)x_out, (float*)h, mean, rstd, M, T, eps, affine);                   \
    else                                                                                                                       \
      hipLaunchKernelGGL((add_ln_mod_fwd16_kernel<bf16_t, NCH>), dim3(g16), dim3(256), 0, st, (const bf16_t*)x_in,            \
                         (const bf16_t*)y, gate, shift, scale, mod_ld, (bf16_t*)x_out, (bf16_t*)h, mean, rstd, M, T, eps,       \
                         affine);                                                                                               \
    break;
    switch (D / 128) {
      F16_CASE(1) F16_CASE(2) F16_CASE(3) F16_CASE(4) F16_CASE(5) F16_CASE(6) F16_CASE(7) F16_CASE(8) F16_CASE(9) F16_CASE(10)
      F16_CASE(11) F16_CASE(12)
    }
#undef F16_CASE
    const double e = dtype == UWU_BF16 ? 2.0 : 4.0, md = (double)M * D;
    prof.done(UWU_PROF_LN_FWD, dtype == UWU_BF16 ? 0 : 1, 8.0 * md, md * e * (2 + (y ? 1 : 0) + (x_out && x_out != x_in ? 1 : 0)));
    UWU_LAUNCH_CHECK("add_ln_modulate_fwd");
    return UWU_OK;
  }
#define FWD_CASE(NIT)                                                                                              \
  case NIT:                                                                                                        \
    if (dtype == UWU_F32)                                                                                          \
      hipLaunchKernelGGL((add_ln_mod_fwd_kernel<float, NIT>), dim3(grid), dim3(256), 0, st, (const float*)x_in,    \
                         (const float*)y, gate, shift, scale, mod_ld, (float*)x_out, (float*)h, mean, rstd, M, T, D, \
                         eps, affine);                                                                                     \
    else                                                                                                           \
      hipLaunchKernelGGL((add_ln_mod_fwd_kernel<bf16_t, NIT>), dim3(grid), dim3(256), 0, st, (const bf16_t*)x_in,  \
                         (const bf16_t*)y, gate, shift, scale, mod_ld, (bf16_t*)x_out, (bf16_t*)h, mean, rstd, M,  \
                         T, D, eps, affine);                                                                               \
    break;
  switch ((D + 511) / 512) {
    FWD_CASE(1) FWD_CASE(2) FWD_CASE(3) FWD_CASE(4) FWD_CASE(5) FWD_CASE(6) FWD_CASE(7) FWD_CASE(8)
  }
#undef FWD_CASE
  {
    const double e = dtype == UWU_BF16 ? 2.0 : 4.0, md = (double)M * D;
    prof.done(UWU_PROF_LN_FWD, dtype == UWU_BF16 ? 0 : 1, 8.0 * md, md * e * (2 + (y ? 1 : 0) + (x_out && x_out != x_in ? 1 : 0)));
  }
  UWU_LAUNCH_CHECK("add_ln_modulate_fwd");
  return UWU_OK;
}

extern "C" int uwu_add_ln_modulate_bwd(const void* dh, const void* x, const float* mean, const float* rstd,
                                       const float* scale, const void* dx_in, const void* y, const float* gate,
                                       int mod_ld, void* dx_out, void* dy, float* dshift, float* dscale, float* dgate,
                                       int B, int T, int D, int affine, int dtype, void* stream) {
  UWU_CHECK_ARG(dh && x && mean && rstd && dx_out, "add_ln_modulate_bwd: null pointer");
  UWU_CHECK_ARG(B > 0 && T > 0 && D > 0 && D % 8 == 0 && D <= MAX_D, "add_ln_modulate_bwd: D=%d unsupported", D);
  UWU_CHECK_ARG((((uintptr_t)dh | (uintptr_t)x | (uintptr_t)dx_out) & 15) == 0, "add_ln_modulate_bwd: tensors must be 16-byte aligned");
  UWU_CHECK_ARG((y == nullptr) || (gate && dy), "add_ln_modulate_bwd: y needs gate and dy");
  UWU_CHECK_ARG(!(scale || y) || mod_ld % 4 == 0, "add_ln_modulate_bwd: mod_ld must be a multiple of 4");
  const int M = B * T;
  hipStream_t st = (hipStream_t)stream;
  UWU_CHECK_ARG(dtype == UWU_F32 || dtype == UWU_BF16, "add_ln_modulate_bwd: bad dtype");
  if (affine && mod_ld == 0 && scale && !y && dshift && dscale && D <= 2048 && (dx_in == nullptr || ((uintptr_t)dx_in & 15) == 0)) {
    const int rpb = M >= 16384 ? 64 : (M >= 4096 ? 32 : 16);
    const int grid = (M + rpb - 1) / rpb;
    const size_t lds2 = (size_t)8 * 2 * D * sizeof(float);
    if (lds2 > 64 * 1024) {
      static unsigned char done[2][4][UWU_MAX_DEV];
      for (int nit = 1; nit <= 4; ++nit) {
        const void* kf = nullptr;
        if (dtype == UWU_F32)
          kf = nit == 1 ? (const void*)ln_affine_bwd_kernel<float, 1> : nit == 2 ? (const void*)ln_affine_bwd_kernel<float, 2>
               : nit == 3 ? (const void*)ln_affine_bwd_kernel<float, 3> : (const void*)ln_affine_bwd_kernel<float, 4>;
        else
          kf = nit == 1 ? (const void*)ln_affine_bwd_kernel<bf16_t, 1> : nit == 2 ? (const void*)ln_affine_bwd_kernel<bf16_t, 2>
               : nit == 3 ? (const void*)ln_affine_bwd_kernel<bf16_t, 3> : (const void*)ln_affine_bwd_kernel<bf16_t, 4>;
        if (!uwu_func_lds(kf, 160 * 1024, done[dtype == UWU_F32][nit - 1])) {
          uwu_set_error("ln_affine_bwd: the device cannot give a workgroup %d bytes of LDS", 160 * 1024);
          return UWU_ELAUNCH;
        }
      }
    }
    UwuProfScope prof(stream);
#define AFF_CASE(NIT)                                                                                                   \
  case NIT:                                                                                                             \
    if (dtype == UWU_F32)                                                                                               \
      hipLaunchKernelGGL((ln_affine_bwd_kernel<float, NIT>), dim3(grid), dim3(512), lds2, st, (const float*)dh,         \
                         (const float*)x, mean, rstd, scale, (const float*)dx_in, (float*)dx_out, dshift, dscale, M, D, \
                         rpb);                                                                                          \
    else                                                                                                                \
      hipLaunchKernelGGL((ln_affine_bwd_kernel<bf16_t, NIT>), dim3(grid), dim3(512), lds2, st, (const bf16_t*)dh,       \
                         (const bf16_t*)x, mean, rstd, scale, (const bf16_t*)dx_in, (bf16_t*)dx_out, dshift, dscale, M, \
                         D, rpb);                                                                                       \
    break;
    switch ((D + 511) / 512) {
      AFF_CASE(1) AFF_CASE(2) AFF_CASE(3) AFF_CASE(4)
    }
#undef AFF_CASE
    const double e = dtype == UWU_BF16 ? 2.0 : 4.0, md = (double)M * D;
    prof.done(UWU_PROF_LN_BWD, dtype == UWU_BF16 ? 0 : 1, 16.0 * md, md * e * (3 + (dx_in ? 1 : 0)));
    UWU_LAUNCH_CHECK("ln_affine_bwd");
    return UWU_OK;
  }
  int rows = 32;
  while (rows > 1 && T % rows) rows >>= 1;
  const bool small = M / rows < 1024 && T % 16 == 0 && D <= 640;
  if (small) rows = 16;
  while (!small && rows > 4 && M / rows < 1024) rows >>= 1;
  const size_t lds = (size_t)(small ? 8 : (D > 1024 ? 1 : 4)) * 3 * D * sizeof(float);
  if (small) {
    UwuProfScope prof(stream);
#define SMALL_CASE(NIT)                                                                                                \
  case NIT:                                                                                                            \
    hipLaunchKernelGGL((add_ln_mod_bwd_kernel<bf16_t, NIT, 8>), dim3(M / rows), dim3(512), lds, st, (const bf16_t*)dh, \
                       (const bf16_t*)x, mean, rstd, scale, (const bf16_t*)dx_in, (const bf16_t*)y, gate, mod_ld,      \
                       (bf16_t*)dx_out, (bf16_t*)dy, dshift, dscale, dgate, M, T, D, rows, affine);                    \
    break;
    if (dtype == UWU_BF16) {
      switch ((D + 511) / 512) { SMALL_CASE(1) SMALL_CASE(2) }
#undef SMALL_CASE
      const double md = (double)M * D;
      prof.done(UWU_PROF_LN_BWD, 0, 16.0 * md, md * 2.0 * (3 + (dx_in ? 1 : 0) + (y ? 2 : 0)));
      UWU_LAUNCH_CHECK("add_ln_modulate_bwd");
      return UWU_OK;
    }
  }
  UWU_CHECK_ARG(lds <= 160 * 1024, "add_ln_modulate_bwd: D=%d needs %zu B of LDS (> 160 KB)", D, lds);
  UwuProfScope prof(stream);
#define BWD_CASE(NIT)                                                                                               \
  case NIT:                                                                                                         \
    if (lds > 64 * 1024) {                      \
      static unsigned char done[2][UWU_MAX_DEV];                                                                    \
      const void* kf = dtype == UWU_F32 ? reinterpret_cast<const void*>(add_ln_mod_bwd_kernel<float, NIT>)          \
                                        : reinterpret_cast<const void*>(add_ln_mod_bwd_kernel<bf16_t, NIT>);        \
      if (!uwu_func_lds(kf, 160 * 1024, done[dtype == UWU_F32])) {                                                  \
        uwu_set_error("add_ln_modulate_bwd: the device cannot give a workgroup %d bytes of LDS", 160 * 1024);       \
        return UWU_ELAUNCH;                                                                                         \
      }                                                                                                             \
    }                                                                                                               \
    if (dtype == UWU_F32)                                                                                           \
      hipLaunchKernelGGL((add_ln_mod_bwd_kernel<float, NIT>), dim3(M / rows), dim3(256), lds, st, (const float*)dh, \
                         (const float*)x, mean, rstd, scale, (const float*)dx_in, (const float*)y, gate, mod_ld,    \
                         (float*)dx_out, (float*)dy, dshift, dscale, dgate, M, T, D, rows, affine);                         \
    else                                                                                                            \
      hipLaunchKernelGGL((add_ln_mod_bwd_kernel<bf16_t, NIT>), dim3(M / rows), dim3(256), lds, st,                  \
                         (const bf16_t*)dh, (const bf16_t*)x, mean, rstd, scale, (const bf16_t*)dx_in,              \
                         (const bf16_t*)y, gate, mod_ld, (bf16_t*)dx_out, (bf16_t*)dy, dshift, dscale, dgate, M, T,   \
                         D, rows, affine);                                                                                  \
    break;
  switch ((D + 511) / 512) {
    BWD_CASE(1) BWD_CASE(2) BWD_CASE(3) BWD_CASE(4) BWD_CASE(5) BWD_CASE(6)
    default:
      UWU_CHECK_ARG(false, "add_ln_modulate_bwd: D=%d > 3072 not instantiated", D);
  }
#undef BWD_CASE
  {
    const double e = dtype == UWU_BF16 ? 2.0 : 4.0, md = (double)M * D;
    prof.done(UWU_PROF_LN_BWD, dtype == UWU_BF16 ? 0 : 1, 16.0 * md, md * e * (3 + (dx_in ? 1 : 0) + (y ? 2 : 0)));
  }
  UWU_LAUNCH_CHECK("add_ln_modulate_bwd");
  return UWU_OK;
}

static int colsum_impl(const void* X, int dtype, int batch, int M, int N, int ldx, float* out, int accumulate,
                       void* stream);
extern "C" int uwu_colsum(const void* X, int dtype, int M, int N, int ldx, float* out, int accumulate, void* stream) {
  return colsum_impl(X, dtype, 1, M, N, ldx, out, accumulate, stream);
}
extern "C" int uwu_colsum_batched(const void* X, int dtype, int batch, int M, int N, int ldx, float* out,
                                  int accumulate, void* stream) {
  return colsum_impl(X, dtype, batch, M, N, ldx, out, accumulate, stream);
}
static int colsum_impl(const void* X, int dtype, int batch, int M, int N, int ldx, float* out, int accumulate,
                       void* stream) {
  UWU_CHECK_ARG(X && out && batch > 0 && M > 0 && N > 0 && N % 4 == 0 && ldx % 4 == 0 && ldx >= N,
                "colsum: bad args (N=%d ldx=%d)", N, ldx);
  hipStream_t st = (hipStream_t)stream;
  if (!accumulate) {
    if (hipMemsetAsync(out, 0, (size_t)batch * N * sizeof(float), st) != hipSuccess) {
      uwu_set_error("colsum: memset failed");
      return UWU_ELAUNCH;
    }
  }
  int splits = (M + 255) / 256;
  const int strips = (N + 63) / 64;
  int want = 1024 / (strips * batch);
  if (want < 1) want = 1;
  if (splits > want) splits = want;
  const int rows = (M + splits - 1) / splits;
  splits = (M + rows - 1) / rows;
  if (dtype == UWU_F32)
    hipLaunchKernelGGL((colsum_kernel<float>), dim3(strips, splits, batch), dim3(256), 0, st, (const float*)X, M, N, ldx,
                       out, rows);
  else if (dtype == UWU_BF16)
    hipLaunchKernelGGL((colsum_kernel<bf16_t>), dim3(strips, splits, batch), dim3(256), 0, st, (const bf16_t*)X, M, N,
                       ldx, out, rows);
  else
    UWU_CHECK_ARG(false, "colsum: bad dtype");
  UWU_LAUNCH_CHECK("colsum");
  return UWU_OK;
}
```

uwudiff_amd/csrc/skinny.hip:

```cpp
#include "common.h"

namespace {

constexpr int SK_MAX_LDS = 128 * 1024;

__device__ __forceinline__ float silu_f32(float v) { return v / (1.f + __expf(-v)); }

template <int MT, int NPW, int EPI>
__global__ void __launch_bounds__(256) skinny_fwd_kernel(const float* __restrict__ X, const float* __restrict__ W,
                                                         const float* __restrict__ bias, float* __restrict__ Y,
                                                         float* __restrict__ Y2, int M, int N, int K) {
  extern __shared__ __attribute__((aligned(16))) float xs[];
  const int tid = threadIdx.x, lane = tid & 63, wave = tid >> 6;
  for (int i = tid; i < (M * K) >> 2; i += 256) reinterpret_cast<f32x4*>(xs)[i] = reinterpret_cast<const f32x4*>(X)[i];
  __syncthreads();
  const int n0 = (blockIdx.x * 4 + wave) * NPW;
  if (n0 >= N) return;
  float acc[NPW][MT];
#pragma unroll
  for (int j = 0; j < NPW; ++j)
#pragma unroll
    for (int m = 0; m < MT; ++m) acc[j][m] = 0.f;
  for (int k = lane; k < K; k += 64) {
    float w[NPW];
#pragma unroll
    for (int j = 0; j < NPW; ++j) w[j] = (n0 + j < N) ? W[(int64_t)(n0 + j) * K + k] : 0.f;
#pragma unroll
    for (int m = 0; m < MT; ++m) {
      const float x = m < M ? xs[m * K + k] : 0.f;
#pragma unroll
      for (int j = 0; j < NPW; ++j) acc[j][m] += w[j] * x;
    }
  }
#pragma unroll
  for (int j = 0; j < NPW; ++j) {
    const int n = n0 + j;
    if (n >= N) break;
    const float b = EPI != UWU_EPI_NONE ? bias[n] : 0.f;
#pragma unroll
    for (int m = 0; m < MT; ++m) {
      const float v = wave_sum(acc[j][m]) + b;
      if (lane == 0 && m < M) {
        Y[(int64_t)m * N + n] = v;
        if (EPI == UWU_EPI_BIAS_SILU) Y2[(int64_t)m * N + n] = silu_f32(v);
      }
    }
  }
}

template <int R, int KC>
__global__ void __launch_bounds__(256) skinny_dgrad_kernel(const float* __restrict__ dY, const float* __restrict__ W,
                                                           float* __restrict__ dX, int M, int N, int K, int NS) {
  extern __shared__ __attribute__((aligned(16))) float dys[];
  const int tid = threadIdx.x, lane = tid & 63, wave = tid >> 6;
  const int n0 = blockIdx.x * NS;
  const int ns = min(NS, N - n0);
  for (int i = tid; i < M * NS; i += 256) {
    const int m = i / NS, n = i - m * NS;
    dys[i] = n < ns ? dY[(int64_t)m * N + n0 + n] : 0.f;
  }
  __syncthreads();
  float acc[R][KC];
#pragma unroll
  for (int r = 0; r < R; ++r)
#pragma unroll
    for (int c = 0; c < KC; ++c) acc[r][c] = 0.f;
#pragma unroll 2
  for (int n = 0; n < ns; ++n) {
    float w[KC];
#pragma unroll
    for (int c = 0; c < KC; ++c) w[c] = (c * 64 + lane < K) ? W[(int64_t)(n0 + n) * K + c * 64 + lane] : 0.f;
#pragma unroll
    for (int r = 0; r < R; ++r) {
      const int m = wave + 4 * r;
      const float d = m < M ? dys[m * NS + n] : 0.f;
#pragma unroll
      for (int c = 0; c < KC; ++c) acc[r][c] += d * w[c];
    }
  }
#pragma unroll
  for (int r = 0; r < R; ++r) {
    const int m = wave + 4 * r;
    if (m >= M) break;
#pragma unroll
    for (int c = 0; c < KC; ++c)
      if (c * 64 + lane < K) atomicAdd(dX + (int64_t)m * K + c * 64 + lane, acc[r][c]);
  }
}

__global__ void __launch_bounds__(256) skinny_wgrad_kernel(const float* __restrict__ dY, const float* __restrict__ X,
                                                           float* __restrict__ dW, float* __restrict__ db, int M, int N,
                                                           int K) {
  extern __shared__ __attribute__((aligned(16))) float sm[];
  float* xs = sm;
  float* dys = sm + M * K;
  const int tid = threadIdx.x, lane = tid & 63, wave = tid >> 6;
  const int n0 = blockIdx.x * 16;
  for (int i = tid; i < (M * K) >> 2; i += 256) reinterpret_cast<f32x4*>(xs)[i] = reinterpret_cast<const f32x4*>(X)[i];
  for (int i = tid; i < M * 16; i += 256) {
    const int m = i >> 4, j = i & 15;
    dys[i] = n0 + j < N ? dY[(int64_t)m * N + n0 + j] : 0.f;
  }
  __syncthreads();
  const int nb = n0 + 4 * wave;
  for (int k = lane; k < K; k += 64) {
    float a0 = 0.f, a1 = 0.f, a2 = 0.f, a3 = 0.f;
    for (int m = 0; m < M; ++m) {
      const float x = xs[m * K + k];
      const f32x4 d = *reinterpret_cast<const f32x4*>(dys + m * 16 + 4 * wave);
      a0 += d[0] * x;
      a1 += d[1] * x;
      a2 += d[2] * x;
      a3 += d[3] * x;
    }
    if (nb + 0 < N) dW[(int64_t)(nb + 0) * K + k] += a0;
    if (nb + 1 < N) dW[(int64_t)(nb + 1) * K + k] += a1;
    if (nb + 2 < N) dW[(int64_t)(nb + 2) * K + k] += a2;
    if (nb + 3 < N) dW[(int64_t)(nb + 3) * K + k] += a3;
  }
  if (db && lane < 4 && nb + lane < N) {
    float s = 0.f;
    for (int m = 0; m < M; ++m) s += dys[m * 16 + 4 * wave + lane];
    db[nb + lane] += s;
  }
}

#define SK_ALLOW_LDS(kern)                                                                                                  \
  do {                                                                                                                      \
    static unsigned char done_[UWU_MAX_DEV];                                                                                \
    if (!uwu_func_lds(reinterpret_cast<const void*>(kern), SK_MAX_LDS, done_)) {                                           \
      uwu_set_error("skinny_linear: the device cannot give a workgroup %d bytes of LDS", SK_MAX_LDS);                      \
      return UWU_ELAUNCH;                                                                                                   \
    }                                                                                                                       \
  } while (0)

bool aligned16(const void* p) { return (reinterpret_cast<uintptr_t>(p) & 15) == 0; }

}

extern "C" int uwu_skinny_linear_ok(int M, int N, int K) {
  return M >= 1 && M <= 64 && N >= 1 && K >= 4 && K % 4 == 0 && (size_t)M * K * sizeof(float) + (size_t)M * 64 <= SK_MAX_LDS;
}

extern "C" int uwu_skinny_linear_fwd(const float* X, const float* W, const float* bias, float* Y, float* Y2, int M, int N,
                                     int K, int epilogue, void* stream) {
  UWU_CHECK_ARG(X && W && Y, "skinny_linear_fwd: null pointer");
  UWU_CHECK_ARG(uwu_skinny_linear_ok(M, N, K), "skinny_linear_fwd: M=%d N=%d K=%d not covered", M, N, K);
  UWU_CHECK_ARG(epilogue == UWU_EPI_NONE || epilogue == UWU_EPI_BIAS || epilogue == UWU_EPI_BIAS_SILU,
                "skinny_linear_fwd: epilogue %d", epilogue);
  UWU_CHECK_ARG(epilogue == UWU_EPI_NONE || bias, "skinny_linear_fwd: bias missing");
  UWU_CHECK_ARG(epilogue != UWU_EPI_BIAS_SILU || Y2, "skinny_linear_fwd: second output missing");
  UWU_CHECK_ARG(aligned16(X), "skinny_linear_fwd: X must be 16-byte aligned");
  hipStream_t st = (hipStream_t)stream;
  const size_t lds = (size_t)M * K * sizeof(float);
  UwuProfScope prof(stream);
#define SK_FWD(MT, NPW, EPI)                                                                                          \
  do {                                                                                                                \
    auto kern = skinny_fwd_kernel<MT, NPW, EPI>;                                                                      \
    SK_ALLOW_LDS(kern);                                                                                               \
    hipLaunchKernelGGL(kern, dim3((N + 4 * NPW - 1) / (4 * NPW)), dim3(256), lds, st, X, W, bias, Y, Y2, M, N, K);    \
  } while (0)
#define SK_FWD_E(MT, NPW)                                                   \
  do {                                                                      \
    if (epilogue == UWU_EPI_NONE) SK_FWD(MT, NPW, UWU_EPI_NONE);            \
    else if (epilogue == UWU_EPI_BIAS) SK_FWD(MT, NPW, UWU_EPI_BIAS);       \
    else SK_FWD(MT, NPW, UWU_EPI_BIAS_SILU);                                \
  } while (0)
  if (M <= 16) SK_FWD_E(16, 4);
  else if (M <= 32) SK_FWD_E(32, 2);
  else SK_FWD_E(64, 1);
#undef SK_FWD_E
#undef SK_FWD
  prof.done(UWU_PROF_OTHER, 1, 2.0 * M * N * K, ((double)N * K + (double)M * K + (double)M * N) * 4);
  UWU_LAUNCH_CHECK("skinny_linear_fwd");
  return UWU_OK;
}

extern "C" int uwu_skinny_linear_dgrad(const float* dY, const float* W, float* dX, int M, int N, int K, void* stream) {
  UWU_CHECK_ARG(dY && W && dX, "skinny_linear_dgrad: null pointer");
  UWU_CHECK_ARG(M >= 1 && M <= 64 && N >= 1 && K >= 1 && K <= 512, "skinny_linear_dgrad: M=%d N=%d K=%d not covered", M, N, K);
  hipStream_t st = (hipStream_t)stream;
  if (hipMemsetAsync(dX, 0, (size_t)M * K * sizeof(float), st) != hipSuccess) {
    uwu_set_error("skinny_linear_dgrad: memset failed");
    return UWU_ELAUNCH;
  }
  int NS = (N / 96 + 15) & ~15;
  if (NS > 16 * M) NS = 16 * M;
  if (NS > ((SK_MAX_LDS / 4 / M) & ~15)) NS = (SK_MAX_LDS / 4 / M) & ~15;
  if (NS < 16) NS = 16;
  const int grid = (N + NS - 1) / NS;
  const size_t lds = (size_t)M * NS * sizeof(float);
  UwuProfScope prof(stream);
#define SK_DG(R, KC)                                                                                  \
  do {                                                                                                \
    auto kern = skinny_dgrad_kernel<R, KC>;                                                           \
    SK_ALLOW_LDS(kern);                                                                               \
    hipLaunchKernelGGL(kern, dim3(grid), dim3(256), lds, st, dY, W, dX, M, N, K, NS);                 \
  } while (0)
#define SK_DG_K(R)                    \
  do {                                \
    if (K <= 256) SK_DG(R, 4);        \
    else if (K <= 384) SK_DG(R, 6);   \
    else SK_DG(R, 8);                 \
  } while (0)
  if (M <= 16) SK_DG_K(4);
  else if (M <= 32) SK_DG_K(8);
  else SK_DG_K(16);
#undef SK_DG_K
#undef SK_DG
  prof.done(UWU_PROF_OTHER, 1, 2.0 * M * N * K, ((double)N * K + (double)M * K + (double)M * N) * 4);
  UWU_LAUNCH_CHECK("skinny_linear_dgrad");
  return UWU_OK;
}

extern "C" int uwu_skinny_linear_wgrad(const float* dY, const float* X, float* dW, float* db, int M, int N, int K,
                                       void* stream) {
  UWU_CHECK_ARG(dY && X && dW, "skinny_linear_wgrad: null pointer");
  UWU_CHECK_ARG(uwu_skinny_linear_ok(M, N, K), "skinny_linear_wgrad: M=%d N=%d K=%d not covered", M, N, K);
  UWU_CHECK_ARG(aligned16(X), "skinny_linear_wgrad: X must be 16-byte aligned");
  hipStream_t st = (hipStream_t)stream;
  const size_t lds = (size_t)M * K * sizeof(float) + (size_t)M * 16 * sizeof(float);
  SK_ALLOW_LDS(skinny_wgrad_kernel);
  UwuProfScope prof(stream);
  hipLaunchKernelGGL(skinny_wgrad_kernel, dim3((N + 15) / 16), dim3(256), lds, st, dY, X, dW, db, M, N, K);
  prof.done(UWU_PROF_OTHER, 1, 2.0 * M * N * K, ((double)N * K * 2 + (double)M * K + (double)M * N) * 4);
  UWU_LAUNCH_CHECK("skinny_linear_wgrad");
  return UWU_OK;
}
```

uwudiff_amd/lib.py:

```python
import ctypes
import os
from ctypes import c_char_p, c_float, c_int, c_int32, c_int64, c_size_t, c_void_p

import torch

_HERE = os.path.dirname(os.path.abspath(__file__))
LIB_PATH = os.path.join(_HERE, "libuwu_hip.so")

F32, BF16 = 0, 1
PT = {"epsilon": 0, "v_prediction": 1, "sample": 2, "rectified_flow": 3}
EPI_NONE, EPI_BIAS, EPI_BIAS_GELU, EPI_DGELU, EPI_BIAS_SILU, EPI_ACCUM = 0, 1, 2, 3, 4, 5
ACT = {"quick_gelu": 0, "gelu": 1}
GATE = {"gated-gelu": 0}


class UwuError(RuntimeError):
    pass


class DitDesc(ctypes.Structure):
    _fields_ = (
        [(n, c_int32) for n in ("B", "T", "D", "H", "L", "mlp_ratio", "in_ch", "out_ch", "patch", "img", "dtype",
                                "cond_dim", "freq_dim")]
        + [("ln_eps", c_float), ("mod_total", c_int32)]
        + [("w", c_void_p), ("w32", c_void_p), ("g32", c_void_p)]
        + [(n, c_int64) for n in ("off_patch_w", "off_patch_b", "off_t_w1", "off_t_b1", "off_t_w2", "off_t_b2",
                                  "off_y_w", "off_y_b", "off_mod_w", "off_mod_b", "off_final_w", "off_final_b",
                                  "off_layer0", "layer_stride")]
        + [("pos", c_void_p), ("ws", c_void_p), ("ws_bytes", c_size_t), ("layer_done", c_void_p)]
        + [("side_stream", c_void_p)]
        + [("rope", c_int32), ("off_rope_h", c_int64), ("off_rope_w", c_int64), ("pos_xy", c_void_p)]
        + [("fp8", c_int32), ("f8_scale", c_void_p), ("f8_amax", c_void_p), ("f8_fmt", c_void_p)]
        + [("checkpoint", c_int32)]
    )


P = c_void_p
_SIGS = {
    "uwu_last_error": (c_char_p, []),
    "uwu_version": (c_int, []),
    "uwu_env_refresh": (c_int, []),
    "uwu_memset_zero": (c_int, [P, ctypes.c_uint64, P]),
    "uwu_schedule_gather": (c_int, [P, P, P, P, c_int, c_int, c_int, c_float, c_int, P, P]),
    "uwu_rf_time_to_sigma": (c_int, [P, c_float, P, c_int, c_int, P, P, P]),
    "uwu_qsample": (c_int, [P, P, P, c_int, c_int64, P, P, P]),
    "uwu_philox_raw": (c_int, [P, c_int64, ctypes.c_uint64, ctypes.c_uint64, P]),
    "uwu_philox_normal": (c_int, [P, c_int64, ctypes.c_uint64, ctypes.c_uint64, P]),
    "uwu_draw_timesteps": (c_int, [P, c_int, c_int, ctypes.c_uint64, ctypes.c_uint64, P]),
    "uwu_draw_u01": (c_int, [P, c_int, ctypes.c_uint64, ctypes.c_uint64, P]),
    "uwu_qsample_draw": (c_int, [P, P, c_int, c_int64, c_int, c_float, c_float, P, P, P, ctypes.c_uint64, ctypes.c_uint64, P]),
    "uwu_posterior_draw": (c_int, [P, c_int, c_int, c_int, c_int64, P, P, P, ctypes.c_uint64, ctypes.c_uint64, P]),
    "uwu_qsample_norm": (c_int, [P, P, P, c_int, c_int64, c_float, c_float, P, P, P]),
    "uwu_ctx_place": (c_int, [P, c_int, P, P] + [c_int] * 7 + [P]),
    "uwu_loss_fwd_bwd": (c_int, [P, P, P, P, c_int, P, c_int, c_int, c_int, c_int, c_int64, P, P, P, P, P, P]),
    "uwu_scale_inplace": (c_int, [P, c_int, c_int64, P, P]),
    "uwu_scale_into": (c_int, [P, P, c_int, c_int64, P, P]),
    "uwu_cast_i64_to_f32": (c_int, [P, P, c_int64, P]),
    "uwu_sampler_step": (c_int, [P, P, P, P, P, P, c_int64, c_float, c_float, c_float, c_float, c_float, P]),
    "uwu_aggregate_concat": (c_int, [P, P, P, c_int, c_int, c_int64, c_int, ctypes.c_uint64, P]),
    "uwu_aggregate_split": (c_int, [P, P, P, c_int, c_int, c_int64, P]),
    "uwu_aggregate_first": (c_int, [P, P, P, c_int, c_int64, P]),
    "uwu_sampler_combine": (c_int, [P, P, P, P, P, c_int64, c_float, c_float, c_float, c_float, P]),
    "uwu_scale_copy": (c_int, [P, P, c_int64, c_float, P]),
    "uwu_cfg_input": (c_int, [P, P, c_int, c_int64, c_float, P]),
    "uwu_sampler_combine_draw": (c_int, [P, P, P, P, c_int64, c_float, c_float, c_float, c_float, ctypes.c_uint64, ctypes.c_uint64, P]),
    "uwu_latent_finish_ws_bytes": (ctypes.c_size_t, [c_int, c_int64]),
    "uwu_latent_finish": (c_int, [P, P, c_int, c_int64, c_int, c_float, c_float, P, ctypes.c_size_t, P]),
    "uwu_image_u8": (c_int, [P, c_int, P, c_int, c_int, c_int, P]),
    "uwu_grad_sqnorm_clip": (c_int, [P, c_int64, c_float, c_float, P, P, P]),
    "uwu_adamw_step": (c_int, [P, P, P, P, P, c_int64, c_float, c_float, c_float, c_float, c_float, c_int, c_float,
                               P, c_int, P]),
    "uwu_cast_f32_to_bf16": (c_int, [P, P, c_int64, P]),
    "uwu_cast_bf16_to_f32": (c_int, [P, P, c_int64, P]),
    "uwu_adapter_merge": (c_int, [P, P, P, P, c_int, c_int64, P, P, P]),
    "uwu_adapter_grad": (c_int, [P, c_int64, c_int64, c_int, P, P, c_int64, c_int64, c_int64, c_int, c_int, c_int, c_float,
                                 P, c_int64, P]),
    "uwu_comm_unique_id": (c_int, [P]),
    "uwu_comm_init": (c_int, [P, c_int, c_int, ctypes.POINTER(c_void_p)]),
    "uwu_allreduce_flat": (c_int, [P, P, c_int64, P]),
    "uwu_comm_destroy": (c_int, [P]),
    "uwu_gemm": (c_int, [P, P, P, P, P, P] + [c_int] * 13 + [P]),
    "uwu_gemm_fp8_scratch_bytes": (ctypes.c_size_t, [c_int, c_int, c_int]),
    "uwu_gemm_fp8": (c_int, [P, P, P, P, P, P] + [c_int] * 9 + [P, P, P, ctypes.c_size_t, P]),
    "uwu_fp8_amax": (c_int, [P, c_int, c_int64, P, P]),
    "uwu_fp8_update_scales": (c_int, [P, P, P, c_int, c_float, P]),
    "uwu_fp8_quantize": (c_int, [P, c_int, c_int, c_int, c_int, P, c_int, P, c_int, P, c_int, P, P, P]),
    "uwu_gemm_fp8_emit": (c_int, [P, P, P, P, P, P, c_int, c_int, c_int, c_int, c_int, c_int, c_int, c_int, c_int, P, P, P, c_int, P, c_int, P,
                                  P, P]),
    "uwu_gemm_wgrad_scratch_bytes": (ctypes.c_size_t, [c_int, c_int, c_int]),
    "uwu_gemm_wgrad": (c_int, [P, P, P, P] + [c_int] * 8 + [P, ctypes.c_size_t, P]),
    "uwu_gemm_wgrad_pair_scratch_bytes": (ctypes.c_size_t, [c_int] * 5),
    "uwu_gemm_wgrad_pair": (c_int, ([P, P, P, P] + [c_int] * 5) * 2 + [c_int] * 3 + [P, ctypes.c_size_t, P]),
    "uwu_gemm_prof_enable": (c_int, [c_int]),
    "uwu_gemm_prof_collect": (c_int, [c_int, P, P, P]),
    "uwu_prof_enable": (c_int, [c_int]),
    "uwu_prof_collect": (c_int, [c_int, c_int, P, P, P, P]),
    "uwu_colsum": (c_int, [P, c_int, c_int, c_int, c_int, P, c_int, P]),
    "uwu_colsum_batched": (c_int, [P, c_int, c_int, c_int, c_int, c_int, P, c_int, P]),
    "uwu_skinny_linear_ok": (c_int, [c_int, c_int, c_int]),
    "uwu_skinny_linear_fwd": (c_int, [P, P, P, P, P, c_int, c_int, c_int, c_int, P]),
    "uwu_skinny_linear_dgrad": (c_int, [P, P, P, c_int, c_int, c_int, P]),
    "uwu_skinny_linear_wgrad": (c_int, [P, P, P, P, c_int, c_int, c_int, P]),
    "uwu_add_ln_modulate_fwd": (c_int, [P, P, P, P, P, c_int, P, P, P, P, c_int, c_int, c_int, c_float, c_int, c_int, P]),
    "uwu_add_ln_modulate_fwd_q8": (c_int, [P, P, P, P, P, c_int, P, P, c_int, P, c_int, P, P, P, P, c_int, c_int, c_int, c_float, P]),
    "uwu_add_ln_modulate_bwd": (c_int, [P, P, P, P, P, P, P, P, c_int, P, P, P, P, P, c_int, c_int, c_int, c_int, c_int, P]),
    "uwu_attention_fwd": (c_int, [P, P, P, P, P] + [c_int] * 9 + [c_float, c_int, P]),
    "uwu_attention_d512_fwd": (c_int, [P, P, P, P] + [c_int] * 6 + [c_float, c_int, P]),
    "uwu_attention_causal_fwd": (c_int, [P] * 5 + [c_int] * 8 + [c_float, c_int, P]),
    "uwu_text_embed": (c_int, [P, P, P, P, c_int, c_int, c_int, c_int, c_int, P]),
    "uwu_bias_act_fwd": (c_int, [P, P, P, c_int, c_int, c_int, c_int, c_int, P]),
    "uwu_text_pool": (c_int, [P, P, P, c_int, c_int, c_int, c_int, c_int, P]),
    "uwu_attention_relbias_fwd": (c_int, [P] * 6 + [c_int] * 8 + [c_float, c_int, P]),
    "uwu_add_rmsnorm_fwd": (c_int, [P] * 5 + [c_int, c_int, c_float, c_int, P]),
    "uwu_gated_act_fwd": (c_int, [P, P] + [c_int] * 6 + [P]),
    "uwu_t5_rel_bias": (c_int, [P, P, P, c_int, c_int, c_int, P]),
    "uwu_token_embed": (c_int, [P, P, P, c_int, c_int, c_int, c_int, c_int, P]),
    "uwu_attention_bwd": (c_int, [P] * 10 + [c_int] * 9 + [c_float, c_int, P]),
    "uwu_attention_bias_fwd": (c_int, [P] * 6 + [c_int] * 9 + [c_float, c_int, P]),
    "uwu_attention_bias_bwd": (c_int, [P] * 11 + [c_int] * 9 + [c_float, c_int, P]),
    "uwu_axial_rope_fwd": (c_int, [P, P, P, P, P, c_int64, c_int, c_int, c_int, c_int, P]),
    "uwu_axial_rope_bwd": (c_int, [P, P, P, P, P, P, P, P, c_int64, c_int, c_int, c_int, c_int, P]),
    "uwu_axial_rope_bwd_shared": (c_int, [P, P, P, c_int, P, P, P, P, P, c_int64, c_int, c_int, c_int, c_int, P]),
    "uwu_axial_rope_table": (c_int, [P, P, P, P, c_int, c_int, c_int, c_int, P]),
    "uwu_attention_rope_fwd": (c_int, [P] * 6 + [c_int] * 9 + [c_float, c_int, P]),
    "uwu_attention_rope_bwd": (c_int, [P] * 10 + [c_int] * 9 + [c_float, c_int, P]),
    "uwu_timestep_embedding": (c_int, [P, c_int, c_int, c_float, P, c_int, P]),
    "uwu_silu_fwd": (c_int, [P, P, c_int64, c_int, P]),
    "uwu_silu_bwd": (c_int, [P, P, P, c_int64, c_int, P]),
    "uwu_add": (c_int, [P, P, P, c_int64, c_int, P]),
    "uwu_transpose_bf16": (c_int, [P, P, c_int, c_int, c_int, c_int, P]),
    "uwu_patchify": (c_int, [P, P, c_int, c_int, c_int, c_int, c_int, c_int, P]),
    "uwu_unpatchify": (c_int, [P, c_int, P, c_int, c_int, c_int, c_int, c_int, P]),
    "uwu_add_pos": (c_int, [P, P, c_int, c_int, c_int, c_int, P]),
    "uwu_groupnorm_fwd": (c_int, [P, P, P, P, P, P, c_int, c_int, c_int, c_int, c_float, c_int, c_int, P]),
    "uwu_groupnorm_fwd_det_ws_bytes": (ctypes.c_size_t, [c_int] * 4),
    "uwu_groupnorm_fwd_det": (c_int, [P, P, P, P, P, P, P, ctypes.c_size_t, c_int, c_int, c_int, c_int, c_float, c_int, c_int, P]),
    "uwu_groupnorm_bwd": (c_int, [P] * 10 + [c_int] * 6 + [P]),
    "uwu_im2col3x3": (c_int, [P, P] + [c_int] * 6 + [P]),
    "uwu_col2im3x3": (c_int, [P, P] + [c_int] * 6 + [P]),
    "uwu_conv3x3_implicit_ok": (c_int, [c_int] * 7),
    "uwu_conv3x3_fwd": (c_int, [P, P, P, P] + [c_int] * 7 + [P]),
    "uwu_conv3x3_s2br_ws_bytes": (ctypes.c_size_t, [c_int] * 6),
    "uwu_conv3x3_s2br_fwd": (c_int, [P, P, P, P] + [c_int] * 6 + [P, ctypes.c_size_t, P]),
    "uwu_conv3x3_dgrad": (c_int, [P, P, P] + [c_int] * 7 + [P]),
    "uwu_conv3x3_wgrad_scratch_bytes": (ctypes.c_size_t, [c_int, c_int, c_int64]),
    "uwu_conv3x3_wgrad": (c_int, [P, P, P, P] + [c_int] * 7 + [P, ctypes.c_size_t, P]),
    "uwu_geglu_fwd": (c_int, [P, P, c_int64, c_int, c_int, P]),
    "uwu_geglu_bwd": (c_int, [P, P, P, c_int64, c_int, c_int, P]),
    "uwu_upsample2x": (c_int, [P, P] + [c_int] * 6 + [P]),
    "uwu_add_rowvec": (c_int, [P, P, c_int, c_int, c_int, c_int, P]),
    "uwu_nchw_to_cl": (c_int, [P, P, c_int, c_int, c_int, c_int, P]),
    "uwu_cl_to_nchw": (c_int, [P, P, c_int, c_int, c_int, c_int, P]),
    "uwu_dit_workspace_bytes": (c_size_t, [ctypes.POINTER(DitDesc)]),
    "uwu_dit_forward": (c_int, [ctypes.POINTER(DitDesc), P, P, P, P, P]),
    "uwu_dit_backward": (c_int, [ctypes.POINTER(DitDesc), P, P]),
    "uwu_dit_backward_cond": (c_int, [ctypes.POINTER(DitDesc), P, P]),
    "uwu_dit_layer_param_stride": (c_int64, [c_int, c_int]),
}

_lib = None


def exported_symbols():
    return sorted(_SIGS)


def load():
    global _lib
    if _lib is not None:
        return _lib
    if not os.path.exists(LIB_PATH):
        raise UwuError(
            f"{LIB_PATH} not found: build it with `python -m uwudiff_amd.build` "
            "(the HIP extension is required; there is no fallback path)"
        )
    lib = ctypes.CDLL(LIB_PATH)
    for name, (res, args) in _SIGS.items():
        fn = getattr(lib, name)
        fn.restype = res
        fn.argtypes = args
    _lib = lib
    return lib


def check(rc, what=""):
    if rc != 0:
        msg = load().uwu_last_error().decode(errors="replace")
        raise UwuError(f"{what} failed (code {rc}): {msg}")


def dt(t: torch.Tensor) -> int:
    if t.dtype == torch.float32:
        return F32
    if t.dtype == torch.bfloat16:
        return BF16
    raise UwuError(f"unsupported dtype {t.dtype}")


def ptr(t):
    if t is None:
        return None
    if not t.is_cuda:
        raise UwuError("libuwu_hip kernels need device tensors (got a CPU tensor); there is no CPU path")
    if not t.is_contiguous():
        raise UwuError("libuwu_hip kernels need contiguous tensors")
    return t.data_ptr()


def stream():
    return torch.cuda.current_stream().cuda_stream


def call(name, *args):
    lib = load()
    rc = getattr(lib, name)(*args)
    check(rc, name)
```

Baseline: 17530 images/s.

## Add batch fp32 linear kernels, batched fc2 transpose, fused cast-colsum, vectorized colsum

Adds a split-K fp32 tiled GEMM for medium-batch conditioning linears (M 64..1024, N<=512), used for timestep/conditioning MLP forward, dgrad and wgrad with a fused bias gradient. Hoists all per-layer fc2 weight transposes into one batched transpose launch before the backward loop, at the cost of extra memory for L transposed copies. Fuses the dmod fp32-to-bf16 cast with its column sum. Widens the bf16 colsum to 8-wide loads with unrolled rows and folds narrow columns. These target launch overhead and small-kernel inefficiency in the conditioning path and backward pass.

After: 17670 images/s (median of 6 runs). Within noise of the previous version (+0.8%).

```diff
diff --git a/include/uwu_hip.h b/include/uwu_hip.h
--- a/include/uwu_hip.h
+++ b/include/uwu_hip.h
@@ -176,6 +176,12 @@
                           int epilogue, void* stream);
 int uwu_skinny_linear_dgrad(const float* dY, const float* W, float* dX, int M, int N, int K, void* stream);
 int uwu_skinny_linear_wgrad(const float* dY, const float* X, float* dW, float* db, int M, int N, int K, void* stream);
+int uwu_batch_linear_ok(int M, int N, int K);
+int uwu_batch_linear_fwd(const float* X, const float* W, const float* bias, float* Y, float* Y2, int M, int N, int K,
+                         int epilogue, void* stream);
+int uwu_batch_linear_dgrad(const float* dY, const float* W, float* dX, int M, int N, int K, void* stream);
+int uwu_batch_linear_wgrad(const float* dY, const float* X, float* dW, float* db, int M, int N, int K, void* stream);
+int uwu_cast_colsum_f32_bf16(const float* X, void* X16, int M, int N, float* out, int accumulate, void* stream);
 int uwu_colsum_batched(const void* X, int dtype, int batch, int M, int N, int ldx, float* out, int accumulate,
                        void* stream);
 
@@ -249,6 +255,8 @@
 
 int uwu_add(const void* a, const void* b, void* out, int64_t n, int dtype, void* stream);
 int uwu_transpose_bf16(const void* src, void* dst, int rows, int cols, int ld_src, int ld_dst, void* stream);
+int uwu_transpose_bf16_batched(const void* src, void* dst, int rows, int cols, int ld_src, int ld_dst, int batch,
+                               int64_t src_stride, int64_t dst_stride, void* stream);
 
 int uwu_patchify(const float* img, void* tok, int B, int C, int H, int W, int p, int dtype, void* stream);
 int uwu_unpatchify(const void* tok, int dtype, float* img, int B, int C, int H, int W, int p, void* stream);
diff --git a/uwudiff_amd/csrc/dit.cpp b/uwudiff_amd/csrc/dit.cpp
--- a/uwudiff_amd/csrc/dit.cpp
+++ b/uwudiff_amd/csrc/dit.cpp
@@ -20,7 +20,7 @@
   size_t sc16, dmod16;
   size_t tok, xe;
   size_t layer0, layer_stride;
-  bool ckpt;
+  bool ckpt, w2t_all;
   size_t keep, scratch0;
   size_t o_x0, o_m1, o_r1, o_h1, o_qkv, o_lse, o_ao, o_y1, o_x1, o_m2, o_r2, o_h2, o_u, o_f, o_y2;
   size_t o_rope;
@@ -100,7 +100,8 @@
   L.dqkv = take(L.M * L.D3 * L.es);
   L.dao = take(L.M * L.D * L.es);
   L.du = take(L.M * L.D4 * L.es);
-  L.w2t = take((size_t)L.D4 * d.D * 2);
+  L.w2t_all = d.dtype == UWU_BF16 && !d.fp8 && !d.checkpoint;
+  L.w2t = take((size_t)L.D4 * d.D * 2 * (L.w2t_all ? d.L : 1));
   L.delta = take((size_t)d.B * d.H * d.T * f4);
   L.dotok = take(L.M * L.Ko * L.es);
   L.dmod = take((size_t)d.B * d.mod_total * f4);
@@ -176,6 +177,7 @@
 }
 int lin_fwd32(const float* X, const float* W, const float* bias, float* Y, float* Y2, int M, int N, int K, int epi, void* st) {
   if (M <= 16 && N <= 4096 && uwu_skinny_linear_ok(M, N, K)) return uwu_skinny_linear_fwd(X, W, bias, Y, Y2, M, N, K, epi, st);
+  if (uwu_batch_linear_ok(M, N, K)) return uwu_batch_linear_fwd(X, W, bias, Y, Y2, M, N, K, epi, st);
   return lin_fwd(X, W, bias, Y, Y2, M, N, K, UWU_F32, UWU_F32, epi, st);
 }
 int lin_dgrad(const void* dY, const void* W, void* dX, const void* aux, int M, int N, int K, int dt, void* st,
@@ -228,6 +230,7 @@
 
 int lin_wgrad32(const float* dY, const float* X, float* dW, float* db, int M, int N, int K, void* st) {
   if (M <= 16 && uwu_skinny_linear_ok(M, N, K)) return uwu_skinny_linear_wgrad(dY, X, dW, db, M, N, K, st);
+  if (uwu_batch_linear_ok(M, N, K)) return uwu_batch_linear_wgrad(dY, X, dW, db, M, N, K, st);
   RUN(lin_wgrad(dY, X, dW, M, N, K, UWU_F32, st));
   return uwu_colsum(dY, UWU_F32, M, N, N, db, 1, st);
 }
@@ -582,6 +585,10 @@
   const bool pair_fc = pairs && wgrad_pair_ok(M, D4, D, D, D4, L.wsc_bytes);
   const bool pair_attn = pairs && wgrad_pair_ok(M, D3, D, D, D, L.wsc_bytes);
 
+  const bool fc2_as = !d.fp8 && dt == UWU_BF16 && D == 384 && M % 256 == 0 && M >= 256 * 256 && D4 % 64 == 0 && D4 >= 1024 && D4 <= 2048;
+  if (fc2_as && L.w2t_all)
+    RUN(uwu_transpose_bf16_batched(layer_weights(d, 0).fc2_w, P.at(L.w2t), D, D4, D4, D, d.L, d.layer_stride, (int64_t)D4 * D, st));
+
   RUN(uwu_patchify(dout, P.at(L.dotok), B, d.out_ch, d.img, d.img, d.patch, dt, st));
   RUN(lin_wgrad(P.at(L.dotok), P.at(L.hF), g + d.off_final_w, M, (int)L.Ko, D, dt, st));
   RUN(uwu_colsum(P.at(L.dotok), dt, M, (int)L.Ko, (int)L.Ko, g + d.off_final_b, 1, st));
@@ -620,9 +627,10 @@
     side_used[0] = true;
     }
     if (side_used[1]) RUN(join_side(fk, 1));
-    if (dt == UWU_BF16 && D == 384 && M % 256 == 0 && M >= 256 * 256 && D4 % 64 == 0 && D4 >= 1024 && D4 <= 2048) {
-      RUN(uwu_transpose_bf16(w.fc2_w, P.at(L.w2t), D, D4, D4, D, st));
-      RUN(uwu_gemm(P.at(L.dy), P.at(L.w2t), P.at(L.du), nullptr, nullptr, P.lay(l, L.o_u), M, D4, D, D, D, D4, D4, 0, 0, dt, dt,
+    if (fc2_as) {
+      char* w2t = P.at<char>(L.w2t) + (L.w2t_all ? (size_t)l * D4 * D * 2 : 0);
+      if (!L.w2t_all) RUN(uwu_transpose_bf16(w.fc2_w, w2t, D, D4, D4, D, st));
+      RUN(uwu_gemm(P.at(L.dy), w2t, P.at(L.du), nullptr, nullptr, P.lay(l, L.o_u), M, D4, D, D, D, D4, D4, 0, 0, dt, dt,
                    UWU_EPI_DGELU, 1, st));
     } else {
       RUN(lin_dgrad(P.at(L.dy), w.fc2_w, P.at(L.du), P.lay(l, L.o_u), M, D, D4, dt, st, nullptr));
@@ -713,9 +721,8 @@
   RUN(uwu_colsum(P.at(L.dx), dt, M, D, D, g + d.off_patch_b, 1, st));
 
   if (mod_bf16(d)) {
-    RUN(uwu_cast_f32_to_bf16(dmod, P.at(L.dmod16), (int64_t)B * ML, st));
+    RUN(uwu_cast_colsum_f32_bf16(dmod, P.at(L.dmod16), B, ML, g + d.off_mod_b, 1, st));
     RUN(lin_wgrad(P.at(L.dmod16), P.at(L.sc16), g + d.off_mod_w, B, ML, D, UWU_BF16, st));
-    RUN(uwu_colsum(dmod, UWU_F32, B, ML, ML, g + d.off_mod_b, 1, st));
     if (hipMemsetAsync(P.at(L.dsc), 0, (size_t)B * D * sizeof(float), (hipStream_t)st) != hipSuccess) {
       uwu_set_error("dit_backward: memset failed");
       return UWU_ELAUNCH;
@@ -737,6 +744,7 @@
   }
   RUN(lin_wgrad32(P.at<float>(L.dc), P.at<float>(L.t_h), g + d.off_t_w2, g + d.off_t_b2, B, D, D, st));
   if (B <= 16 && uwu_skinny_linear_ok(B, D, D) && D <= 512) RUN(uwu_skinny_linear_dgrad(P.at<float>(L.dc), w32 + d.off_t_w2, P.at<float>(L.dth), B, D, D, st));
+  else if (uwu_batch_linear_ok(B, D, D)) RUN(uwu_batch_linear_dgrad(P.at<float>(L.dc), w32 + d.off_t_w2, P.at<float>(L.dth), B, D, D, st));
   else RUN(lin_dgrad(P.at(L.dc), w32 + d.off_t_w2, P.at(L.dth), nullptr, B, D, D, UWU_F32, st));
   RUN(uwu_silu_bwd(P.at(L.t_pre), P.at(L.dth), P.at(L.dtp), (int64_t)B * D, UWU_F32, st));
   RUN(lin_wgrad32(P.at<float>(L.dtp), P.at<float>(L.feat), g + d.off_t_w1, g + d.off_t_b1, B, D, d.freq_dim, st));
diff --git a/uwudiff_amd/csrc/embed.hip b/uwudiff_amd/csrc/embed.hip
--- a/uwudiff_amd/csrc/embed.hip
+++ b/uwudiff_amd/csrc/embed.hip
@@ -157,8 +157,11 @@
 
 namespace {
 __global__ void __launch_bounds__(256) transpose_bf16_kernel(const bf16_t* __restrict__ src, bf16_t* __restrict__ dst, int rows,
-                                                             int cols, int lds, int ldd) {
+                                                             int cols, int lds, int ldd, int64_t src_stride,
+                                                             int64_t dst_stride) {
   __shared__ bf16_t tile[32][34];
+  src += blockIdx.z * src_stride;
+  dst += blockIdx.z * dst_stride;
   const int tx = threadIdx.x & 31, ty = threadIdx.x >> 5;
   const int r0 = blockIdx.y * 32, c0 = blockIdx.x * 32;
 #pragma unroll
@@ -178,7 +181,18 @@
 extern "C" int uwu_transpose_bf16(const void* src, void* dst, int rows, int cols, int ld_src, int ld_dst, void* stream) {
   UWU_CHECK_ARG(src && dst && rows > 0 && cols > 0 && ld_src >= cols && ld_dst >= rows, "transpose_bf16: bad argument");
   hipLaunchKernelGGL(transpose_bf16_kernel, dim3((cols + 31) / 32, (rows + 31) / 32), dim3(256), 0, (hipStream_t)stream,
-                     (const bf16_t*)src, (bf16_t*)dst, rows, cols, ld_src, ld_dst);
+                     (const bf16_t*)src, (bf16_t*)dst, rows, cols, ld_src, ld_dst, (int64_t)0, (int64_t)0);
   UWU_LAUNCH_CHECK("transpose_bf16");
   return UWU_OK;
 }
+
+extern "C" int uwu_transpose_bf16_batched(const void* src, void* dst, int rows, int cols, int ld_src, int ld_dst, int batch,
+                                          int64_t src_stride, int64_t dst_stride, void* stream) {
+  UWU_CHECK_ARG(src && dst && rows > 0 && cols > 0 && ld_src >= cols && ld_dst >= rows, "transpose_bf16_batched: bad argument");
+  UWU_CHECK_ARG(batch > 0 && batch <= 65535 && src_stride >= 0 && dst_stride >= (int64_t)(cols - 1) * ld_dst + rows,
+                "transpose_bf16_batched: bad batch / stride");
+  hipLaunchKernelGGL(transpose_bf16_kernel, dim3((cols + 31) / 32, (rows + 31) / 32, batch), dim3(256), 0, (hipStream_t)stream,
+                     (const bf16_t*)src, (bf16_t*)dst, rows, cols, ld_src, ld_dst, src_stride, dst_stride);
+  UWU_LAUNCH_CHECK("transpose_bf16_batched");
+  return UWU_OK;
+}
diff --git a/uwudiff_amd/csrc/norm.hip b/uwudiff_amd/csrc/norm.hip
--- a/uwudiff_amd/csrc/norm.hip
+++ b/uwudiff_amd/csrc/norm.hip
@@ -547,28 +547,78 @@
   }
 }
 
-template <typename T>
+template <int V>
+struct ColVec;
+template <>
+struct ColVec<4> {
+  typedef f32x4 type;
+  template <typename T>
+  static __device__ __forceinline__ f32x4 load(const T* p) { return load4(p); }
+};
+template <>
+struct ColVec<8> {
+  typedef f32x8 type;
+  template <typename T>
+  static __device__ __forceinline__ f32x8 load(const T* p) { return load8(p); }
+};
+template <typename T, int V = 4, bool CAST = false>
 __global__ void __launch_bounds__(256) colsum_kernel(const T* __restrict__ X, int M, int N, int ldx,
-                                                     float* __restrict__ out, int rows_per_block) {
-  __shared__ f32x4 red[16][17];
+                                                     float* __restrict__ out, int rows_per_block, int nout,
+                                                     bf16_t* __restrict__ X16) {
+  typedef typename ColVec<V>::type vec;
+  __shared__ float red[16][16 * V + 4];
   const int cg = threadIdx.x & 15, rg = threadIdx.x >> 4;
-  const int n = blockIdx.x * 64 + cg * 4;
+  const int n0 = blockIdx.x * 16 * V, n = n0 + cg * V;
   X += (int64_t)blockIdx.z * M * ldx;
-  out += (int64_t)blockIdx.z * N;
+  out += (int64_t)blockIdx.z * nout;
   const int r0 = blockIdx.y * rows_per_block;
   int r1 = r0 + rows_per_block;
   if (r1 > M) r1 = M;
-  f32x4 a = {0.f, 0.f, 0.f, 0.f};
-  if (n < N)
-    for (int r = r0 + rg; r < r1; r += 16) a = a + load4(X + (int64_t)r * ldx + n);
-  red[rg][cg] = a;
+  vec a = {};
+  if (n < N) {
+    vec b = {}, c = {}, d = {};
+    int r = r0 + rg;
+    for (; r + 48 < r1; r += 64) {
+      const int64_t o = (int64_t)r * ldx + n;
+      const vec v0 = ColVec<V>::load(X + o), v1 = ColVec<V>::load(X + o + 16 * (int64_t)ldx),
+                v2 = ColVec<V>::load(X + o + 32 * (int64_t)ldx), v3 = ColVec<V>::load(X + o + 48 * (int64_t)ldx);
+      if constexpr (CAST) {
+        store4(X16 + o, v0);
+        store4(X16 + o + 16 * (int64_t)ldx, v1);
+        store4(X16 + o + 32 * (int64_t)ldx, v2);
+        store4(X16 + o + 48 * (int64_t)ldx, v3);
+      }
+      a = a + v0;
+      b = b + v1;
+      c = c + v2;
+      d = d + v3;
+    }
+    for (; r < r1; r += 16) {
+      const vec v = ColVec<V>::load(X + (int64_t)r * ldx + n);
+      if constexpr (CAST) store4(X16 + (int64_t)r * ldx + n, v);
+      a = a + v;
+    }
+    a = (a + b) + (c + d);
+  }
+#pragma unroll
+  for (int e = 0; e < V; ++e) red[rg][cg * V + e] = a[e];
   __syncthreads();
-  if (rg == 0 && n < N) {
-    f32x4 t = red[0][cg];
-#pragma unroll
-    for (int i = 1; i < 16; ++i) t = t + red[i][cg];
-#pragma unroll
-    for (int e = 0; e < 4; ++e) atomicAdd(out + n + e, t[e]);
+  const int t = threadIdx.x;
+  if (t < 16 * V) {
+    float s = red[0][t];
+#pragma unroll
+    for (int i = 1; i < 16; ++i) s += red[i][t];
+    red[0][t] = s;
+  }
+  if (nout >= N) {
+    if (t < 16 * V && n0 + t < N) atomicAdd(out + n0 + t, red[0][t]);
+    return;
+  }
+  __syncthreads();
+  if (t < nout) {
+    float s = red[0][t];
+    for (int k = t + nout; k < 16 * V; k += nout) s += red[0][k];
+    atomicAdd(out + t, s);
   }
 }
 
@@ -813,21 +863,53 @@
       return UWU_ELAUNCH;
     }
   }
+  const bool v8 = dtype == UWU_BF16 && N % 8 == 0 && ldx % 8 == 0 && (((uintptr_t)X) & 15) == 0;
+  const int W = v8 ? 128 : 64;
+  const int nout = N;
+  const bool fold = batch == 1 && N < W && W % N == 0 && ldx == N && M % (W / N) == 0 && (((uintptr_t)X) & 15) == 0;
+  if (fold) {
+    M /= W / N;
+    N = ldx = W;
+  }
   int splits = (M + 255) / 256;
-  const int strips = (N + 63) / 64;
-  int want = 1024 / (strips * batch);
+  const int strips = (N + W - 1) / W;
+  int want = (fold ? 96 : 1024) / (strips * batch);
   if (want < 1) want = 1;
   if (splits > want) splits = want;
   const int rows = (M + splits - 1) / splits;
   splits = (M + rows - 1) / rows;
   if (dtype == UWU_F32)
     hipLaunchKernelGGL((colsum_kernel<float>), dim3(strips, splits, batch), dim3(256), 0, st, (const float*)X, M, N, ldx,
-                       out, rows);
+                       out, rows, nout, (bf16_t*)nullptr);
+  else if (dtype == UWU_BF16 && v8)
+    hipLaunchKernelGGL((colsum_kernel<bf16_t, 8>), dim3(strips, splits, batch), dim3(256), 0, st, (const bf16_t*)X, M, N,
+                       ldx, out, rows, nout, (bf16_t*)nullptr);
   else if (dtype == UWU_BF16)
     hipLaunchKernelGGL((colsum_kernel<bf16_t>), dim3(strips, splits, batch), dim3(256), 0, st, (const bf16_t*)X, M, N,
-                       ldx, out, rows);
+                       ldx, out, rows, nout, (bf16_t*)nullptr);
   else
     UWU_CHECK_ARG(false, "colsum: bad dtype");
   UWU_LAUNCH_CHECK("colsum");
   return UWU_OK;
 }
+
+extern "C" int uwu_cast_colsum_f32_bf16(const float* X, void* X16, int M, int N, float* out, int accumulate, void* stream) {
+  UWU_CHECK_ARG(X && X16 && out && M > 0 && N > 0 && N % 4 == 0, "cast_colsum: bad args (M=%d N=%d)", M, N);
+  UWU_CHECK_ARG((((uintptr_t)X) & 15) == 0 && (((uintptr_t)X16) & 7) == 0, "cast_colsum: misaligned tensor");
+  hipStream_t st = (hipStream_t)stream;
+  if (!accumulate && hipMemsetAsync(out, 0, (size_t)N * sizeof(float), st) != hipSuccess) {
+    uwu_set_error("cast_colsum: memset failed");
+    return UWU_ELAUNCH;
+  }
+  const int strips = (N + 63) / 64;
+  int splits = (M + 63) / 64;
+  int want = 2048 / strips;
+  if (want < 1) want = 1;
+  if (splits > want) splits = want;
+  const int rows = (M + splits - 1) / splits;
+  splits = (M + rows - 1) / rows;
+  hipLaunchKernelGGL((colsum_kernel<float, 4, true>), dim3(strips, splits, 1), dim3(256), 0, st, X, M, N, N, out, rows, N,
+                     (bf16_t*)X16);
+  UWU_LAUNCH_CHECK("cast_colsum");
+  return UWU_OK;
+}
diff --git a/uwudiff_amd/csrc/skinny.hip b/uwudiff_amd/csrc/skinny.hip
--- a/uwudiff_amd/csrc/skinny.hip
+++ b/uwudiff_amd/csrc/skinny.hip
@@ -122,6 +122,126 @@
     float s = 0.f;
     for (int m = 0; m < M; ++m) s += dys[m * 16 + 4 * wave + lane];
     db[nb + lane] += s;
+  }
+}
+
+constexpr int BL_T = 32, BL_K = 64, BL_LD = 36;
+constexpr int BL_NW = 8, BL_NT = 64 * BL_NW;
+constexpr int BL_ACC = 100;
+
+template <bool TR>
+__device__ __forceinline__ f32x4 bl_load(const float* __restrict__ P, int ld, int r0, int k0, int R, int k1, int tid) {
+  if (TR) {
+    const int k = k0 + (tid >> 3), row = r0 + 4 * (tid & 7);
+    if (k < k1 && row < R) return load4(P + (int64_t)k * ld + row);
+  } else {
+    const int row = r0 + (tid >> 4), k = k0 + 4 * (tid & 15);
+    if (row < R && k < k1) return load4(P + (int64_t)row * ld + k);
+  }
+  return f32x4{0.f, 0.f, 0.f, 0.f};
+}
+template <bool TR>
+__device__ __forceinline__ void bl_store(const f32x4& r, float* s, int tid) {
+  if (TR) {
+    store4(s + (tid >> 3) * BL_LD + 4 * (tid & 7), r);
+  } else {
+#pragma unroll
+    for (int e = 0; e < 4; ++e) s[(4 * (tid & 15) + e) * BL_LD + (tid >> 4)] = r[e];
+  }
+}
+
+template <bool TA, bool TB, int EPI>
+__global__ void __launch_bounds__(BL_NT) batch_linear_kernel(const float* __restrict__ A, const float* __restrict__ B,
+                                                             const float* __restrict__ bias, float* __restrict__ C,
+                                                             float* __restrict__ C2, float* __restrict__ db, int M, int N, int K,
+                                                             int lda, int ldb, int ldc, int k_per_split) {
+  constexpr int STAGE = BL_K * BL_LD;
+  constexpr int KW = BL_K / BL_NW;
+  static_assert(4 * STAGE >= BL_NW * 1024 + BL_NW * 32, "the waves' partial tiles reuse the stages");
+  __shared__ __attribute__((aligned(16))) float sm[4 * STAGE];
+  const int tid = threadIdx.x, lane = tid & 63, wave = tid >> 6;
+  const int ty = lane >> 3, tx = lane & 7;
+  const int m0 = blockIdx.y * BL_T, n0 = blockIdx.x * BL_T;
+  const int kb = blockIdx.z * k_per_split;
+  const int k1 = min(K, kb + k_per_split);
+  const bool want_db = EPI == BL_ACC && db != nullptr && blockIdx.x == 0;
+
+  f32x4 acc[2][4];
+#pragma unroll
+  for (int h = 0; h < 2; ++h)
+#pragma unroll
+    for (int i = 0; i < 4; ++i) acc[h][i] = f32x4{0.f, 0.f, 0.f, 0.f};
+  f32x4 asum[2] = {f32x4{0.f, 0.f, 0.f, 0.f}, f32x4{0.f, 0.f, 0.f, 0.f}};
+  f32x4 ra = bl_load<TA>(A, lda, m0, kb, M, k1, tid), rb = bl_load<TB>(B, ldb, n0, kb, N, k1, tid);
+  bl_store<TA>(ra, sm, tid);
+  bl_store<TB>(rb, sm + STAGE, tid);
+  __syncthreads();
+  int cur = 0;
+  for (int k0 = kb; k0 < k1; k0 += BL_K) {
+    const bool more = k0 + BL_K < k1;
+    if (more) {
+      ra = bl_load<TA>(A, lda, m0, k0 + BL_K, M, k1, tid);
+      rb = bl_load<TB>(B, ldb, n0, k0 + BL_K, N, k1, tid);
+    }
+    const float* as = sm + cur * 2 * STAGE + (wave * KW) * BL_LD + 4 * ty;
+    const float* bs = sm + cur * 2 * STAGE + STAGE + (wave * KW) * BL_LD + 4 * tx;
+#pragma unroll
+    for (int kk = 0; kk < KW; ++kk) {
+      const f32x4 a = load4(as + kk * BL_LD), b = load4(bs + kk * BL_LD);
+#pragma unroll
+      for (int i = 0; i < 4; ++i) acc[kk & 1][i] = acc[kk & 1][i] + f32x4{a[i], a[i], a[i], a[i]} * b;
+      if (want_db) asum[kk & 1] = asum[kk & 1] + a;
+    }
+    if (more) {
+      bl_store<TA>(ra, sm + (cur ^ 1) * 2 * STAGE, tid);
+      bl_store<TB>(rb, sm + (cur ^ 1) * 2 * STAGE + STAGE, tid);
+    }
+    __syncthreads();
+    cur ^= 1;
+  }
+  float* red = sm;
+#pragma unroll
+  for (int i = 0; i < 4; ++i) store4(red + wave * 1024 + (4 * ty + i) * 32 + 4 * tx, acc[0][i] + acc[1][i]);
+  if (want_db) {
+    if (tx == 0) store4(red + BL_NW * 1024 + wave * 32 + 4 * ty, asum[0] + asum[1]);
+  }
+  __syncthreads();
+  if (tid < 256) {
+    const int r = tid >> 3, c = 4 * (tid & 7);
+    f32x4 v[BL_NW];
+#pragma unroll
+    for (int w = 0; w < BL_NW; ++w) v[w] = load4(red + w * 1024 + r * 32 + c);
+#pragma unroll
+    for (int st = 1; st < BL_NW; st *= 2)
+#pragma unroll
+      for (int w = 0; w + st < BL_NW; w += 2 * st) v[w] = v[w] + v[w + st];
+    const int m = m0 + r, n = n0 + c;
+    if (m < M && n < N) {
+      float* cp = C + (int64_t)m * ldc + n;
+      if (EPI == BL_ACC) {
+        if (gridDim.z == 1) {
+          store4(cp, load4(cp) + v[0]);
+        } else {
+#pragma unroll
+          for (int e = 0; e < 4; ++e) atomicAdd(cp + e, v[0][e]);
+        }
+      } else {
+        if (EPI != UWU_EPI_NONE) v[0] = v[0] + load4(bias + n);
+        store4(cp, v[0]);
+        if (EPI == UWU_EPI_BIAS_SILU)
+          store4(C2 + (int64_t)m * ldc + n, f32x4{silu_f(v[0][0]), silu_f(v[0][1]), silu_f(v[0][2]), silu_f(v[0][3])});
+      }
+    }
+  } else if (want_db && tid < 256 + 32 && m0 + tid - 256 < M) {
+    const float* p = red + BL_NW * 1024 + tid - 256;
+    float s[BL_NW];
+#pragma unroll
+    for (int w = 0; w < BL_NW; ++w) s[w] = p[32 * w];
+#pragma unroll
+    for (int st = 1; st < BL_NW; st *= 2)
+#pragma unroll
+      for (int w = 0; w + st < BL_NW; w += 2 * st) s[w] = s[w] + s[w + st];
+    atomicAdd(db + m0 + tid - 256, s[0]);
   }
 }
 
@@ -227,3 +347,72 @@
   UWU_LAUNCH_CHECK("skinny_linear_wgrad");
   return UWU_OK;
 }
+
+extern "C" int uwu_batch_linear_ok(int M, int N, int K) {
+  return M >= 64 && M <= 1024 && N >= 4 && N <= 512 && N % 4 == 0 && K >= 4 && K % 4 == 0;
+}
+
+namespace {
+int bl_split(int tiles, int K, int* k_per_split) {
+  const int stages = (K + BL_K - 1) / BL_K;
+  int split = (256 + tiles - 1) / tiles;
+  if (split < (K + 255) / 256) split = (K + 255) / 256;
+  if (split > stages) split = stages;
+  if (split < 1) split = 1;
+  const int per = (stages + split - 1) / split;
+  *k_per_split = per * BL_K;
+  return (stages + per - 1) / per;
+}
+}
+
+extern "C" int uwu_batch_linear_fwd(const float* X, const float* W, const float* bias, float* Y, float* Y2, int M, int N, int K,
+                                    int epilogue, void* stream) {
+  UWU_CHECK_ARG(X && W && Y, "batch_linear_fwd: null pointer");
+  UWU_CHECK_ARG(uwu_batch_linear_ok(M, N, K), "batch_linear_fwd: M=%d N=%d K=%d not covered", M, N, K);
+  UWU_CHECK_ARG(epilogue == UWU_EPI_NONE || epilogue == UWU_EPI_BIAS || epilogue == UWU_EPI_BIAS_SILU,
+                "batch_linear_fwd: epilogue %d", epilogue);
+  UWU_CHECK_ARG(epilogue == UWU_EPI_NONE || bias, "batch_linear_fwd: bias missing");
+  UWU_CHECK_ARG(epilogue != UWU_EPI_BIAS_SILU || Y2, "batch_linear_fwd: second output missing");
+  UWU_CHECK_ARG(aligned16(X) && aligned16(W) && aligned16(Y) && aligned16(Y2) && aligned16(bias),
+                "batch_linear_fwd: tensors must be 16-byte aligned");
+  hipStream_t st = (hipStream_t)stream;
+  const dim3 grid((N + BL_T - 1) / BL_T, (M + BL_T - 1) / BL_T, 1);
+  UwuProfScope prof(stream);
+#define BL_FWD(EPI) \
+  hipLaunchKernelGGL((batch_linear_kernel<false, false, EPI>), grid, dim3(BL_NT), 0, st, X, W, bias, Y, Y2, (float*)nullptr, M, N, K, K, K, N, K)
+  if (epilogue == UWU_EPI_NONE) BL_FWD(UWU_EPI_NONE);
+  else if (epilogue == UWU_EPI_BIAS) BL_FWD(UWU_EPI_BIAS);
+  else BL_FWD(UWU_EPI_BIAS_SILU);
+#undef BL_FWD
+  prof.done(UWU_PROF_OTHER, 1, 2.0 * M * N * K, ((double)N * K + (double)M * K + (double)M * N) * 4);
+  UWU_LAUNCH_CHECK("batch_linear_fwd");
+  return UWU_OK;
+}
+
+extern "C" int uwu_batch_linear_dgrad(const float* dY, const float* W, float* dX, int M, int N, int K, void* stream) {
+  UWU_CHECK_ARG(dY && W && dX, "batch_linear_dgrad: null pointer");
+  UWU_CHECK_ARG(uwu_batch_linear_ok(M, N, K), "batch_linear_dgrad: M=%d N=%d K=%d not covered", M, N, K);
+  UWU_CHECK_ARG(aligned16(dY) && aligned16(W) && aligned16(dX), "batch_linear_dgrad: tensors must be 16-byte aligned");
+  const dim3 grid((K + BL_T - 1) / BL_T, (M + BL_T - 1) / BL_T, 1);
+  UwuProfScope prof(stream);
+  hipLaunchKernelGGL((batch_linear_kernel<false, true, UWU_EPI_NONE>), grid, dim3(BL_NT), 0, (hipStream_t)stream, dY, W,
+                     (const float*)nullptr, dX, (float*)nullptr, (float*)nullptr, M, K, N, N, K, K, N);
+  prof.done(UWU_PROF_OTHER, 1, 2.0 * M * N * K, ((double)N * K + (double)M * K + (double)M * N) * 4);
+  UWU_LAUNCH_CHECK("batch_linear_dgrad");
+  return UWU_OK;
+}
+
+extern "C" int uwu_batch_linear_wgrad(const float* dY, const float* X, float* dW, float* db, int M, int N, int K, void* stream) {
+  UWU_CHECK_ARG(dY && X && dW, "batch_linear_wgrad: null pointer");
+  UWU_CHECK_ARG(uwu_batch_linear_ok(M, N, K), "batch_linear_wgrad: M=%d N=%d K=%d not covered", M, N, K);
+  UWU_CHECK_ARG(aligned16(dY) && aligned16(X) && aligned16(dW), "batch_linear_wgrad: tensors must be 16-byte aligned");
+  dim3 grid((K + BL_T - 1) / BL_T, (N + BL_T - 1) / BL_T, 1);
+  int per = 0;
+  grid.z = bl_split(grid.x * grid.y, M, &per);
+  UwuProfScope prof(stream);
+  hipLaunchKernelGGL((batch_linear_kernel<true, true, BL_ACC>), grid, dim3(BL_NT), 0, (hipStream_t)stream, dY, X,
+                     (const float*)nullptr, dW, (float*)nullptr, db, N, K, M, N, K, K, per);
+  prof.done(UWU_PROF_OTHER, 1, 2.0 * M * N * K, ((double)N * K * 2 + (double)M * K + (double)M * N) * 4);
+  UWU_LAUNCH_CHECK("batch_linear_wgrad");
+  return UWU_OK;
+}
diff --git a/uwudiff_amd/lib.py b/uwudiff_amd/lib.py
--- a/uwudiff_amd/lib.py
+++ b/uwudiff_amd/lib.py
@@ -101,6 +101,11 @@
     "uwu_skinny_linear_fwd": (c_int, [P, P, P, P, P, c_int, c_int, c_int, c_int, P]),
     "uwu_skinny_linear_dgrad": (c_int, [P, P, P, c_int, c_int, c_int, P]),
     "uwu_skinny_linear_wgrad": (c_int, [P, P, P, P, c_int, c_int, c_int, P]),
+    "uwu_batch_linear_ok": (c_int, [c_int, c_int, c_int]),
+    "uwu_batch_linear_fwd": (c_int, [P, P, P, P, P, c_int, c_int, c_int, c_int, P]),
+    "uwu_batch_linear_dgrad": (c_int, [P, P, P, c_int, c_int, c_int, P]),
+    "uwu_batch_linear_wgrad": (c_int, [P, P, P, P, c_int, c_int, c_int, P]),
+    "uwu_cast_colsum_f32_bf16": (c_int, [P, P, c_int, c_int, P, c_int, P]),
     "uwu_add_ln_modulate_fwd": (c_int, [P, P, P, P, P, c_int, P, P, P, P, c_int, c_int, c_int, c_float, c_int, c_int, P]),
     "uwu_add_ln_modulate_fwd_q8": (c_int, [P, P, P, P, P, c_int, P, P, c_int, P, c_int, P, P, P, P, c_int, c_int, c_int, c_float, P]),
     "uwu_add_ln_modulate_bwd": (c_int, [P, P, P, P, P, P, P, P, c_int, P, P, P, P, P, c_int, c_int, c_int, c_int, c_int, P]),
@@ -129,6 +134,7 @@
     "uwu_silu_bwd": (c_int, [P, P, P, c_int64, c_int, P]),
     "uwu_add": (c_int, [P, P, P, c_int64, c_int, P]),
     "uwu_transpose_bf16": (c_int, [P, P, c_int, c_int, c_int, c_int, P]),
+    "uwu_transpose_bf16_batched": (c_int, [P, P, c_int, c_int, c_int, c_int, c_int, c_int64, c_int64, P]),
     "uwu_patchify": (c_int, [P, P, c_int, c_int, c_int, c_int, c_int, c_int, P]),
     "uwu_unpatchify": (c_int, [P, c_int, P, c_int, c_int, c_int, c_int, c_int, P]),
     "uwu_add_pos": (c_int, [P, P, c_int, c_int, c_int, c_int, P]),
```
